# willis-richard/connect4

Hardware: AMD Instinct MI355X
Metric: mcts_node_expansions_per_sec (higher is better)
Workload: dtype f32x3

## Files before the change

### connect4_amd/csrc/c4_engine.hip

```cpp
#include <hip/hip_runtime.h>
#include <hip/hip_fp16.h>
#include <hip/hip_bfloat16.h>

#include <algorithm>
#include <cmath>
#include <cstdarg>
#include <cstdio>
#include <cstdlib>
#include <cstring>
#include <limits>
#include <vector>

#include "../../include/c4_engine.h"
#include "c4_board.h"
#include "c4_net_dev.h"

#ifndef C4_DEADLINE_EVERY
#define C4_DEADLINE_EVERY 1
#endif
#ifndef C4_TERMQ
#define C4_TERMQ 1
#endif
#ifndef C4_FUSED_NET_STAMPS
#define C4_FUSED_NET_STAMPS 0
#endif
#ifndef C4_ASM_PICK
#define C4_ASM_PICK 1
#endif
#ifndef C4_SPECULATE
#define C4_SPECULATE 1
#endif
#ifndef C4_SPLIT_PHASES
#define C4_SPLIT_PHASES 0
#endif
#ifndef C4_DIV_NORMAL
#define C4_DIV_NORMAL 1
#endif
#ifndef C4_SCORE_ALL
#define C4_SCORE_ALL 1
#endif
#ifndef C4_PATH_ALL_LANES
#define C4_PATH_ALL_LANES 1
#endif
#ifndef C4_PEEL_BACKUP
#define C4_PEEL_BACKUP 1
#endif
#ifndef C4_NO_SUSPEND
#define C4_NO_SUSPEND 1
#endif
#ifndef C4_NET_SANITISES
#define C4_NET_SANITISES 1
#endif
#ifndef C4_WAIT_CLOCK_LAZY
#define C4_WAIT_CLOCK_LAZY 1
#endif
#ifndef C4_SPLIT_PAIRS
#define C4_SPLIT_PAIRS 1
#endif
#ifndef C4_SORT_SLOTS
#define C4_SORT_SLOTS 1
#endif
#ifndef C4_FILLERS
#define C4_FILLERS (C4_ORIENTED_Q && C4_SCORE_ALL)
#endif
#ifndef C4_VGPR_BASES
#define C4_VGPR_BASES 1
#endif
#ifndef C4_ORIENTED_Q
#define C4_ORIENTED_Q 1
#endif
#ifndef C4_COOP_LEGAL
#define C4_COOP_LEGAL 1
#endif
#ifndef C4_PICK_BPERM
#define C4_PICK_BPERM 1
#endif
#ifndef C4_EARLY_REQUEST
#define C4_EARLY_REQUEST 1
#endif

namespace {

using namespace c4;

constexpr int GROUP = 8;
constexpr int SLOTS_PER_BLOCK = 8;
constexpr int BLOCK = GROUP * SLOTS_PER_BLOCK;
constexpr int MAX_DEPTH = 44;

constexpr int SLOT_ACTIVE = 0;
constexpr int SLOT_PARKED = 1;
constexpr int SLOT_MOVE_DONE = 2;

__host__ __device__ __forceinline__ uint32_t pack_info(uint32_t base, uint32_t nchild, uint32_t status,
                                                       uint32_t bit, uint32_t pf64)
{
    return (base >> 3) | (nchild << 19) | (status << 22) | (bit << 25) | (pf64 << 31);
}
__host__ __device__ __forceinline__ uint32_t info_base(uint32_t i) { return (i & 0x7ffffu) << 3; }
__host__ __device__ __forceinline__ uint32_t info_nchild(uint32_t i) { return (i >> 19) & 7u; }
__host__ __device__ __forceinline__ uint32_t info_status(uint32_t i) { return (i >> 22) & 7u; }
__host__ __device__ __forceinline__ uint32_t info_bit(uint32_t i) { return (i >> 25) & 63u; }
__host__ __device__ __forceinline__ uint32_t info_move(uint32_t i) { return info_bit(i) / 7u; }
__host__ __device__ __forceinline__ uint32_t info_pf64(uint32_t i) { return i >> 31; }

struct __attribute__((aligned(16))) PathEntry {
    uint32_t node;
    uint32_t n;
    double w;
};

constexpr int BLOCK_BYTES = 256;
struct __attribute__((aligned(32))) Rec {
    double w;
    double q;
    double p;
    uint32_t n;
    uint32_t info;
};
static_assert(sizeof(Rec) == 32, "node record must be 32 bytes");
struct Pool {
    uint8_t *base;
    __device__ __forceinline__ Rec *rec(uint32_t i) const { return reinterpret_cast<Rec *>(base) + i; }
    __device__ __forceinline__ uint32_t &n(uint32_t i) const { return rec(i)->n; }
    __device__ __forceinline__ uint32_t &info(uint32_t i) const { return rec(i)->info; }
    __device__ __forceinline__ double &w(uint32_t i) const { return rec(i)->w; }
    __device__ __forceinline__ double &q(uint32_t i) const { return rec(i)->q; }
    __device__ __forceinline__ double &p(uint32_t i) const { return rec(i)->p; }
};

struct CacheEntry {
    uint64_t key;
    uint64_t check;
    float value;
    float prior[7];
};
static_assert(sizeof(CacheEntry) == 48, "cache entry must be 48 bytes");

struct SlotStats {
    uint64_t sims, expansions, children, terminal_sims, leaf_evals, depth_sum, moves, games_started,
        games_finished, capped, cache_hits, cache_probes, bad_evals, spec_evals;
};
constexpr int N_STATS = sizeof(SlotStats) / sizeof(uint64_t);

struct SlotMem {
    uint64_t root0, root1, leaf0, leaf1;
    long long gid;
    double root_w;
    uint32_t sims, nalloc;
    int32_t pend;
    uint32_t pdepth, pinfo;
    uint32_t ply;
    uint32_t flags;
    __device__ int state() const { return (int)(flags & 0xffu); }
    __device__ bool has_leaf() const { return ((flags >> 8) & 0xffu) != 0; }
    __device__ int need_root() const { return (int)(flags >> 16); }
    __device__ static uint32_t pack(int state, int has_leaf, int need_root) { return (uint32_t)state | ((uint32_t)has_leaf << 8) | ((uint32_t)need_root << 16); }
};
static_assert(sizeof(SlotMem) == 80, "32 of these must fit the fused kernel's LDS budget");

struct Cold {
    uint32_t *cont_cur, *cont_n;
    double *cont_w;
    int32_t *res_move;
    double *res_value;
    double *res_policy;
    const double *noise_tape;
    const double *u_tape;
    int tape_games;
    uint64_t *stg_c0, *stg_c1;
    int32_t *stg_move;
    double *stg_value;
    double *stg_policy;
    c4_game_record *ring;
    unsigned long long *ring_head, *ring_tail, *dropped;
    unsigned long long *next_game;
    unsigned long long *stamps;
};

struct Dev {
    uint8_t *pool;
    uint64_t *root_c0, *root_c1, *leaf_c0, *leaf_c1;
    int32_t *has_leaf;
    int32_t *pending;
    uint32_t *pending_depth;
    uint32_t *pending_info;
    uint32_t *sims_done;
    uint32_t *n_alloc;
    int32_t *state;
    int32_t *need_root;
    uint32_t *ply;
    long long *game_id;
    PathEntry *path;
    uint64_t *stats;
    const double2 *tabAB;
    CacheEntry *cache;
    const Cold *cold;
    int G;
    int slot_lo, slot_hi;
    uint32_t cap;
    int S;
    int nsm;
    int use_noise;
    int rng_tape;
    int stop_after_move;
    int max_inner;
    int level_budget;
    int time_budget;
    int planes_dtype;
    int rec_cap;
    int cache_bits;
    int has_stamps;
    long long games_target;
    double alpha, frac;
    uint64_t seed;
};

__device__ __forceinline__ double gshfl(double v, int src) { return __shfl(v, src, GROUP); }
__device__ __forceinline__ float gshfl(float v, int src) { return __shfl(v, src, GROUP); }
__device__ __forceinline__ int gshfl(int v, int src) { return __shfl(v, src, GROUP); }
__device__ __forceinline__ uint32_t gshfl(uint32_t v, int src) { return (uint32_t)__shfl((int)v, src, GROUP); }

__device__ __forceinline__ void lds_fence() { asm volatile("s_waitcnt lgkmcnt(0)" ::: "memory"); }
typedef __attribute__((address_space(3))) volatile uint32_t lds_vu32_t;
typedef __attribute__((address_space(3))) volatile float lds_vf32_t;
typedef __attribute__((address_space(3))) volatile uint64_t lds_vu64_t;
__device__ __forceinline__ uint32_t lds_ld(const uint32_t *p) { return *(lds_vu32_t *)p; }
__device__ __forceinline__ void lds_st(uint32_t *p, uint32_t v) { *(lds_vu32_t *)p = v; }
__device__ __forceinline__ float lds_ldf(const float *p) { return *(lds_vf32_t *)p; }
__device__ __forceinline__ void lds_st64(uint64_t *p, uint64_t v) { *(lds_vu64_t *)p = v; }

__device__ __forceinline__ void group_fence()
{
    __builtin_amdgcn_fence(__ATOMIC_RELEASE, "workgroup");
    __builtin_amdgcn_fence(__ATOMIC_ACQUIRE, "workgroup");
}

__device__ __forceinline__ void philox_round(uint32_t c[4], const uint32_t k[2])
{
    const uint64_t p0 = (uint64_t)0xD2511F53u * c[0];
    const uint64_t p1 = (uint64_t)0xCD9E8D57u * c[2];
    const uint32_t n0 = (uint32_t)(p1 >> 32) ^ c[1] ^ k[0];
    const uint32_t n1 = (uint32_t)p1;
    const uint32_t n2 = (uint32_t)(p0 >> 32) ^ c[3] ^ k[1];
    const uint32_t n3 = (uint32_t)p0;
    c[0] = n0; c[1] = n1; c[2] = n2; c[3] = n3;
}
__device__ inline void philox4x32(uint32_t c[4], uint64_t seed)
{
    uint32_t k[2] = {(uint32_t)seed, (uint32_t)(seed >> 32)};
#pragma unroll
    for (int r = 0; r < 10; ++r) {
        philox_round(c, k);
        k[0] += 0x9E3779B9u;
        k[1] += 0xBB67AE85u;
    }
}
__device__ inline void rng_uniform2(uint64_t seed, long long gid, uint32_t ply, uint32_t stream, uint32_t idx,
                                    double &u0, double &u1)
{
    uint32_t c[4] = {(uint32_t)gid, (uint32_t)((uint64_t)gid >> 32), ply * 64u + stream, idx};
    philox4x32(c, seed);
    u0 = (double)((((uint64_t)c[0] << 32) | c[1]) >> 11) * (1.0 / 9007199254740992.0);
    u1 = (double)((((uint64_t)c[2] << 32) | c[3]) >> 11) * (1.0 / 9007199254740992.0);
}
__device__ inline double rng_gamma(uint64_t seed, long long gid, uint32_t ply, uint32_t stream, double alpha)
{
    double u0, u1;
    rng_uniform2(seed, gid, ply, stream, 0, u0, u1);
    double boost = 1.0;
    if (alpha < 1.0) {
        boost = pow(u0 > 0.0 ? u0 : 1e-300, 1.0 / alpha);
        alpha += 1.0;
    }
    const double dd = alpha - 1.0 / 3.0, cc = 1.0 / sqrt(9.0 * dd);
    for (uint32_t it = 1; it <= 24; ++it) {
        double a, b, uu, unused;
        rng_uniform2(seed, gid, ply, stream, 2 * it, a, b);
        rng_uniform2(seed, gid, ply, stream, 2 * it + 1, uu, unused);
        const double x = sqrt(-2.0 * log(a > 0.0 ? a : 1e-300)) * cos(6.283185307179586 * b);
        double v = 1.0 + cc * x;
        if (v <= 0.0) continue;
        v = v * v * v;
        if (uu < 1.0 - 0.0331 * x * x * x * x) return boost * dd * v;
        if (log(uu > 0.0 ? uu : 1e-300) < 0.5 * x * x + dd * (1.0 - v + log(v))) return boost * dd * v;
    }
    return boost * dd;
}

__device__ __forceinline__ double child_value_for(uint32_t status, uint32_t n, double q, int side)
{
    const bool term = status >= ST_XWIN;
#if C4_TERMQ
    const double v = q;
#else
    const double v = term ? 0.5 * (double)(status - ST_XWIN) : q;
#endif
    const double sv = side == 0 ? v : 1.0 - v;
    return (term || n > 0) ? sv : 0.0;
}

__device__ __forceinline__ double orient_q(double v, int parent_side)
{
#if C4_ORIENTED_Q
    return (parent_side & 1) ? 1.0 - v : v;
#else
    (void)parent_side;
    return v;
#endif
}

__device__ __forceinline__ double div_normal(double a, double b)
{
#if C4_DIV_NORMAL
    double r = __builtin_amdgcn_rcp(b);
    double e = __builtin_fma(-b, r, 1.0);
    r = __builtin_fma(r, e, r);
    e = __builtin_fma(-b, r, 1.0);
    r = __builtin_fma(r, e, r);
    const double q = a * r;
    const double rem = __builtin_fma(-b, q, a);
    return __builtin_fma(rem, r, q);
#else
    return a / b;
#endif
}

__device__ __forceinline__ double ucb_score(double A, double B, uint32_t nc, double p, double V, uint32_t pf64)
{
    const double pbc = A * div_normal(B, (double)(nc + 1));
    const double prior_score64 = pbc * p;
    const double s64 = prior_score64 + V;
    const float prior_score32 = (float)pbc * (float)p;
    const float s32 = prior_score32 + (float)V;
    return pf64 ? s64 : (double)s32;
}

__device__ __forceinline__ int legal_mask_group(uint64_t occ)
{
#if C4_COOP_LEGAL
    const int lane = (int)(threadIdx.x & (GROUP - 1));
    const bool legal = lane < WIDTH && col_count(occ, lane < WIDTH ? lane : 0) < HEIGHT;
    const unsigned long long b = __builtin_amdgcn_ballot_w64(legal);
    return (int)((b >> (threadIdx.x & 63u & ~(uint32_t)(GROUP - 1))) & 0x7fu);
#else
    return legal_mask(occ);
#endif
}

__device__ __forceinline__ int group_argmax(double s, int k)
{
#pragma unroll
    for (int m = 1; m < GROUP; m <<= 1) {
        const double os = __shfl_xor(s, m, GROUP);
        const int ok = __shfl_xor(k, m, GROUP);
        if (os > s || (os == s && ok > k)) { s = os; k = ok; }
    }
    return k;
}

template <int CTRL>
__device__ __forceinline__ uint32_t dpp_u32(uint32_t v)
{
    return (uint32_t)__builtin_amdgcn_update_dpp(0, (int)v, CTRL, 0xF, 0xF, true);
}
template <int CTRL>
__device__ __forceinline__ double dpp_f64(double v)
{
    const uint64_t b = (uint64_t)__double_as_longlong(v);
    const uint64_t r = ((uint64_t)dpp_u32<CTRL>((uint32_t)(b >> 32)) << 32) | dpp_u32<CTRL>((uint32_t)b);
    return __longlong_as_double((long long)r);
}
struct Pick {
    double s;
    int k;
    uint32_t n, info;
    double w;
};
#define C4_DPP_SELECT(CTRL)                                                                              \
    asm volatile("s_mov_b64 vcc, %[m]\n"                                                                 \
                 "s_nop 0\n"                                                                             \
                 "v_cndmask_b32_dpp %[n], %[n], %[n], vcc " CTRL " row_mask:0xf bank_mask:0xf\n"         \
                 "v_cndmask_b32_dpp %[i], %[i], %[i], vcc " CTRL " row_mask:0xf bank_mask:0xf\n"         \
                 "v_cndmask_b32_dpp %[wl], %[wl], %[wl], vcc " CTRL " row_mask:0xf bank_mask:0xf\n"      \
                 "v_cndmask_b32_dpp %[wh], %[wh], %[wh], vcc " CTRL " row_mask:0xf bank_mask:0xf\n"      \
                 : [n] "+v"(n), [i] "+v"(info), [wl] "+v"(wl), [wh] "+v"(wh)                              \
                 : [m] "s"(m)                                                                             \
                 : "vcc")
#if C4_ASM_PICK
#define C4_PICK_SELECT(CTRL)                                                                             \
    asm volatile("s_mov_b64 vcc, %[m]\n"                                                                 \
                 "s_nop 0\n"                                                                             \
                 "v_cndmask_b32 %[sl], %[ol], %[sl], vcc\n"                                               \
                 "v_cndmask_b32 %[sh], %[oh], %[sh], vcc\n"                                               \
                 "v_cndmask_b32_dpp %[n], %[n], %[n], vcc " CTRL " row_mask:0xf bank_mask:0xf\n"          \
                 "v_cndmask_b32_dpp %[i], %[i], %[i], vcc " CTRL " row_mask:0xf bank_mask:0xf\n"          \
                 "v_cndmask_b32_dpp %[wl], %[wl], %[wl], vcc " CTRL " row_mask:0xf bank_mask:0xf\n"       \
                 "v_cndmask_b32_dpp %[wh], %[wh], %[wh], vcc " CTRL " row_mask:0xf bank_mask:0xf\n"       \
                 : [sl] "+v"(sl), [sh] "+v"(sh), [n] "+v"(n), [i] "+v"(info), [wl] "+v"(wl), [wh] "+v"(wh) \
                 : [m] "s"(m), [ol] "v"(ol), [oh] "v"(oh)                                                   \
                 : "vcc")
template <int CTRL>
__device__ __forceinline__ void pick_step(double &s, uint32_t &n, uint32_t &info, uint32_t &wl, uint32_t &wh)
{
    const uint64_t sb = (uint64_t)__double_as_longlong(s);
    uint32_t sl = (uint32_t)sb, sh = (uint32_t)(sb >> 32);
    const uint32_t ol = dpp_u32<CTRL>(sl), oh = dpp_u32<CTRL>(sh);
    const double os = __longlong_as_double((long long)(((uint64_t)oh << 32) | ol));
    constexpr unsigned long long HIGH = CTRL == 0xB1 ? 0xAAAAAAAAAAAAAAAAull : (CTRL == 0x4E ? 0xCCCCCCCCCCCCCCCCull : 0xF0F0F0F0F0F0F0F0ull);
    const unsigned long long m = __builtin_amdgcn_fcmp(s, os, 2 ) | (__builtin_amdgcn_fcmp(s, os, 3 ) & HIGH);
    if (CTRL == 0xB1) C4_PICK_SELECT("quad_perm:[1,0,3,2]");
    else if (CTRL == 0x4E) C4_PICK_SELECT("quad_perm:[2,3,0,1]");
    else C4_PICK_SELECT("row_half_mirror");
    s = __longlong_as_double((long long)(((uint64_t)sh << 32) | sl));
}
#undef C4_PICK_SELECT
#else
template <int CTRL>
__device__ __forceinline__ void pick_step(double &s, int &k, uint32_t &n, uint32_t &info, uint32_t &wl, uint32_t &wh)
{
    const double os = dpp_f64<CTRL>(s);
    const int ok = (int)dpp_u32<CTRL>((uint32_t)k);
    const bool keep = (s > os) | ((s == os) & (k >= ok));
    s = keep ? s : os;
    k = keep ? k : ok;
    const unsigned long long m = __builtin_amdgcn_ballot_w64(keep);
    if (CTRL == 0xB1) C4_DPP_SELECT("quad_perm:[1,0,3,2]");
    else if (CTRL == 0x4E) C4_DPP_SELECT("quad_perm:[2,3,0,1]");
    else C4_DPP_SELECT("row_half_mirror");
}
#endif
#undef C4_DPP_SELECT
#if C4_PICK_BPERM
__device__ __forceinline__ void group_pick(Pick &a)
{
    double m = a.s, o;
    o = dpp_f64<0xB1>(m);
    asm("v_max_f64 %0, %1, %2" : "=v"(m) : "v"(m), "v"(o));
    o = dpp_f64<0x4E>(m);
    asm("v_max_f64 %0, %1, %2" : "=v"(m) : "v"(m), "v"(o));
    o = dpp_f64<0x141>(m);
    asm("v_max_f64 %0, %1, %2" : "=v"(m) : "v"(m), "v"(o));
    const unsigned long long eq = __builtin_amdgcn_fcmp(a.s, m, 1 );
    const int gb = (int)(threadIdx.x & 63u & ~(uint32_t)(GROUP - 1));
    const uint32_t bits = (uint32_t)(eq >> gb) & 0xffu;
    const int k = 31 - __builtin_clz(bits);
    const int src = (gb + k) << 2;
    const uint64_t wb = (uint64_t)__double_as_longlong(a.w);
    const uint32_t wl = (uint32_t)__builtin_amdgcn_ds_bpermute(src, (int)(uint32_t)wb), wh = (uint32_t)__builtin_amdgcn_ds_bpermute(src, (int)(uint32_t)(wb >> 32));
    a.n = (uint32_t)__builtin_amdgcn_ds_bpermute(src, (int)a.n);
    a.info = (uint32_t)__builtin_amdgcn_ds_bpermute(src, (int)a.info);
    a.w = __longlong_as_double((long long)(((uint64_t)wh << 32) | wl));
    a.k = k;
    a.s = m;
}
#else
__device__ __forceinline__ void group_pick(Pick &a)
{
    const uint64_t wb = (uint64_t)__double_as_longlong(a.w);
    uint32_t wl = (uint32_t)wb, wh = (uint32_t)(wb >> 32);
#if C4_ASM_PICK
    uint32_t nk = a.n | ((uint32_t)(threadIdx.x & (GROUP - 1)) << 29);
    pick_step<0xB1>(a.s, nk, a.info, wl, wh);
    pick_step<0x4E>(a.s, nk, a.info, wl, wh);
    pick_step<0x141>(a.s, nk, a.info, wl, wh);
    a.k = (int)(nk >> 29);
    a.n = nk & 0x1fffffffu;
#else
    pick_step<0xB1>(a.s, a.k, a.n, a.info, wl, wh);
    pick_step<0x4E>(a.s, a.k, a.n, a.info, wl, wh);
    pick_step<0x141>(a.s, a.k, a.n, a.info, wl, wh);
#endif
    a.w = __longlong_as_double((long long)(((uint64_t)wh << 32) | wl));
}
#endif

__device__ __forceinline__ double dirichlet_from_gamma(double nz, bool legal)
{
    if (!legal) nz = 0.0;
    double s = 0.0;
#pragma unroll
    for (int i = 0; i < 7; ++i) s = s + gshfl(nz, i);
    return nz / s;
}

__device__ __forceinline__ int sample_child_sq(double V, bool act, uint32_t nc, double u, int lane)
{
    const double w2 = act ? V * V : 0.0;
    double s2 = 0.0;
#pragma unroll
    for (int i = 0; i < 7; ++i) s2 = s2 + gshfl(w2, i);
    if (!(s2 > 0.0)) return -1;
    const double pk = w2 / s2;
    double acc = 0.0, cdf = 0.0;
#pragma unroll
    for (int i = 0; i < 7; ++i) {
        acc = acc + gshfl(pk, i);
        if (i == lane) cdf = acc;
    }
    const double last = gshfl(cdf, (int)nc - 1);
    cdf = cdf / last;
    const unsigned long long bal = __ballot(act && cdf <= u);
    const int cnt = __popcll((bal >> (((threadIdx.x & 63) / GROUP) * GROUP)) & 0xffull);
    return cnt < (int)nc ? cnt : (int)nc - 1;
}

template <class DevT>
__device__ __forceinline__ void publish_game(DevT &d, int g, long long gid, int len, int32_t result, int lane)
{
    group_fence();
    int ok = 0;
    unsigned long long t = 0;
    if (lane == 0) {
        const unsigned long long tail = *(volatile unsigned long long *)d.cold->ring_tail;
        unsigned long long old = *(volatile unsigned long long *)d.cold->ring_head;
        for (;;) {
            if (old - tail >= (unsigned long long)d.rec_cap) { atomicAdd(d.cold->dropped, 1ULL); break; }
            const unsigned long long seen = atomicCAS(d.cold->ring_head, old, old + 1);
            if (seen == old) { ok = 1; t = old; break; }
            old = seen;
        }
    }
    ok = gshfl(ok, 0);
    if (!ok) return;
    t = ((unsigned long long)gshfl((uint32_t)(t >> 32), 0) << 32) | gshfl((uint32_t)t, 0);
    c4_game_record *row = d.cold->ring + (size_t)(t % (unsigned long long)d.rec_cap);
    const size_t s0 = (size_t)g * 42;
    for (int i = lane; i < len; i += GROUP) {
        row->color0[i] = d.cold->stg_c0[s0 + i];
        row->color1[i] = d.cold->stg_c1[s0 + i];
        row->move[i] = d.cold->stg_move[s0 + i];
        row->value[i] = d.cold->stg_value[s0 + i];
    }
// ... 892 lines not shown
        const int nleaf = sn;
        for (int r0 = 0; r0 < nleaf; r0 += P) {
            if (r0) __syncthreads();
            net_forward_block(nd, NetLds{act, wbuf, mlp}, sleaf[0] + r0, sleaf[1] + r0, min(P, nleaf - r0), 0, s_val, s_pri,
                              smap + r0);
        }
        __syncthreads();
        if (d.has_stamps) t_net += __builtin_amdgcn_s_memtime() - tc;
    }
    if (threadIdx.x < TS && slot0 + threadIdx.x < d.G) {
        const int p = threadIdx.x, g = slot0 + p;
        const SlotMem m = smem[p];
        d.root_c0[g] = m.root0; d.root_c1[g] = m.root1; d.leaf_c0[g] = m.leaf0; d.leaf_c1[g] = m.leaf1;
        d.game_id[g] = m.gid; d.sims_done[g] = m.sims; d.n_alloc[g] = m.nalloc; d.pending[g] = m.pend;
        d.pending_depth[g] = m.pdepth; d.pending_info[g] = m.pinfo; d.need_root[g] = m.need_root();
        d.ply[g] = m.ply; d.state[g] = m.state(); d.has_leaf[g] = m.has_leaf() ? 1 : 0;
    }
    if (threadIdx.x < N_STATS) d.stats[(size_t)slot0 * N_STATS + threadIdx.x] += s_stats[threadIdx.x];
    for (int i = threadIdx.x; i < TS * 8; i += NTHREADS) {
        const int p = i >> 3, k = i & 7;
        if (slot0 + p < d.G) {
            if (k == 7) values[slot0 + p] = s_val[p];
            else priors[(size_t)(slot0 + p) * 7 + k] = s_pri[p * 7 + k];
        }
    }
    if (d.has_stamps && blockIdx.x < 128 && (threadIdx.x & 63) == 0) {
        unsigned long long *o = d.cold->stamps + blockIdx.x * 16;
        o[wv] = t_own;
        if (wv == 0) { o[8] = t_tree; o[9] = t_net; o[10] = (unsigned long long)n_steps; }
    }
}

typedef __attribute__((address_space(4))) const Dev const_dev;
template <int TS, int MODE>
__global__ __launch_bounds__(c4net::NTHREADS) void c4_selfplay_wave_kernel(const Dev *d_dev, c4net::NetDev nd, float *__restrict__ values,
                                                                           float *__restrict__ priors, int n_steps)
{
    using namespace c4net;
    const_dev &d = *(const_dev *)d_dev;
    constexpr int SPW = TS / NWAVES;
    static_assert(TS % NWAVES == 0 && SPW >= 1 && SPW <= 8, "slots per workgroup");
    constexpr int WBUF = WaveBuf<MODE>::HALVES;
    __shared__ __attribute__((aligned(16))) _Float16 act[NWAVES][WBUF];
    __shared__ __attribute__((aligned(16))) float4 mlp[MLP_F4];
    __shared__ SlotMem smem[TS];
    __shared__ float s_val[TS];
    __shared__ float s_pri[TS * 7];
    __shared__ uint32_t s_stats[N_STATS];
    __shared__ __attribute__((aligned(16))) float s_bias[BIAS_LDS_FLOATS];
    __shared__ __attribute__((aligned(16))) uint16_t s_tab16[64 * TAB16];
    constexpr bool OWN_PATH = MODE == NETMODE_F32_F16;
    __shared__ __attribute__((aligned(16))) PathEntry s_path_own[OWN_PATH ? TS : 1][MAX_DEPTH];
    __shared__ __attribute__((aligned(16))) Rec s_l1_own[OWN_PATH ? TS : 1][GROUP];
    static_assert(OWN_PATH || (sizeof(PathEntry) * MAX_DEPTH + sizeof(Rec) * GROUP) * SPW <= sizeof(_Float16) * WBUF, "a wave's path stacks must fit its activation planes");
    const int slot0 = blockIdx.x * TS;
    const int wv = threadIdx.x >> 6;
    if (threadIdx.x < TS) {
        const int p = threadIdx.x, g = slot0 + p;
        SlotMem m = {};
        m.flags = SlotMem::pack(SLOT_PARKED, 0, 0);
        if (g < d.G) {
            m.root0 = d.root_c0[g]; m.root1 = d.root_c1[g]; m.leaf0 = d.leaf_c0[g]; m.leaf1 = d.leaf_c1[g];
            m.gid = d.game_id[g]; m.sims = d.sims_done[g]; m.nalloc = d.n_alloc[g]; m.pend = d.pending[g];
            m.pdepth = d.pending_depth[g]; m.pinfo = d.pending_info[g];
            m.ply = d.ply[g]; m.flags = SlotMem::pack(d.state[g], d.has_leaf[g], d.need_root[g]);
            m.root_w = *(const double *)(d.pool + (size_t)g * d.cap * (BLOCK_BYTES / 8));
        }
        smem[p] = m;
    }
    if (threadIdx.x < N_STATS) s_stats[threadIdx.x] = 0;
    for (int i = threadIdx.x; i < TS * 8; i += NTHREADS) {
        const int p = i >> 3, k = i & 7;
        const bool ok = slot0 + p < d.G;
        if (k == 7) s_val[p] = ok ? values[slot0 + p] : 0.0f;
        else s_pri[p * 7 + k] = ok ? priors[(size_t)(slot0 + p) * 7 + k] : 0.0f;
    }
    for (int i = threadIdx.x; i < MLP_F4; i += NTHREADS) mlp[i] = nd.mlp[i];
    stage_bias_lds(nd, s_bias);
    if (threadIdx.x < 64) build_tab16<MODE == NETMODE_F64 ? CS64 : CS16>(s_tab16, threadIdx.x);
    if (OWN_PATH)
        for (int i = threadIdx.x; i < TS * MAX_DEPTH; i += NTHREADS) {
            const int p = i / MAX_DEPTH, k = i - p * MAX_DEPTH;
            if (slot0 + p < d.G) s_path_own[p][k] = d.path[(size_t)(slot0 + p) * MAX_DEPTH + k];
        }
    __syncthreads();
    PathEntry (*s_path)[MAX_DEPTH] = OWN_PATH ? s_path_own : reinterpret_cast<PathEntry (*)[MAX_DEPTH]>(&act[wv][0]);
    Rec (*s_l1)[GROUP] = OWN_PATH ? s_l1_own : reinterpret_cast<Rec (*)[GROUP]>(&act[wv][0] + sizeof(PathEntry) * MAX_DEPTH * SPW / sizeof(_Float16));
    unsigned long long t_tree = 0, t_net = 0, n_pass = 0;
    const unsigned long long t_launch = __builtin_amdgcn_s_memtime();
    const unsigned long long quantum = (unsigned long long)n_steps * (unsigned long long)(d.time_budget > 0 ? d.time_budget : 80000);
    while (__builtin_amdgcn_s_memtime() - t_launch < quantum) {
        const unsigned long long ta = d.has_stamps ? __builtin_amdgcn_s_memtime() : 0;
        int tid = threadIdx.x;
        asm volatile("" : "+v"(tid));
        const int lane = tid & (GROUP - 1);
        const int grp = (tid & 63) / GROUP;
        const int sl = (tid >> 6) + NWAVES * grp;
        if (grp < SPW)
            tree_step<C4_EVAL_EXTERNAL_F32, false, true, true, OWN_PATH>(d, slot0 + sl, lane, OWN_PATH ? sl : grp, s_path, s_l1, s_val, s_pri, nullptr,
                                                                         nullptr, &smem[sl], sl, s_stats, t_launch + quantum);
        lds_fence();
        const unsigned long long tb = d.has_stamps ? __builtin_amdgcn_s_memtime() : 0;
        int pend_slot[SPW];
        int cnt = 0;
#pragma unroll
        for (int q = 0; q < SPW; ++q) {
            const int sq = wv + NWAVES * q;
            const int has = __builtin_amdgcn_readfirstlane(smem[sq].has_leaf() ? 1 : 0);
            if (has) pend_slot[cnt++] = sq;
        }
        if (MODE == NETMODE_F32_F16) {
            for (int i = 0; i < cnt; ++i) {
                const int sa = pend_slot[i];
                net_forward_wave16(nd, &act[wv][0], mlp, s_bias, s_tab16, smem[sa].leaf0, smem[sa].leaf1, s_val, s_pri, sa,
                                   (C4_FUSED_NET_STAMPS && d.has_stamps && blockIdx.x < 16) ? d.cold->stamps + 2048 + (blockIdx.x * NWAVES + wv) * 16 : nullptr);
            }
        } else {
            for (int i = 0; i < cnt; ++i) {
                const int sa = pend_slot[i];
                net_forward_wave1_mode<MODE>(nd, &act[wv][0], mlp, s_bias, s_tab16, smem[sa].leaf0, smem[sa].leaf1, s_val, s_pri, sa, nd.w0);
            }
        }
        lds_fence();
        if (d.has_stamps) { t_tree += tb - ta; t_net += __builtin_amdgcn_s_memtime() - tb; n_pass += cnt; }
    }
    if (d.has_stamps && blockIdx.x < 128 && (threadIdx.x & 63) == 0) {
        d.cold->stamps[blockIdx.x * 16 + wv] = t_tree;
        d.cold->stamps[blockIdx.x * 16 + 8 + wv] = t_net | (n_pass << 48);
    }
    __syncthreads();
    if (OWN_PATH)
        for (int i = threadIdx.x; i < TS * MAX_DEPTH; i += NTHREADS) {
            const int p = i / MAX_DEPTH, k = i - p * MAX_DEPTH;
            if (slot0 + p < d.G && smem[p].has_leaf()) d.path[(size_t)(slot0 + p) * MAX_DEPTH + k] = s_path_own[p][k];
        }
    if (threadIdx.x < TS && slot0 + threadIdx.x < d.G) {
        const int p = threadIdx.x, g = slot0 + p;
        const SlotMem m = smem[p];
        d.root_c0[g] = m.root0; d.root_c1[g] = m.root1; d.leaf_c0[g] = m.leaf0; d.leaf_c1[g] = m.leaf1;
        d.game_id[g] = m.gid; d.sims_done[g] = m.sims; d.n_alloc[g] = m.nalloc; d.pending[g] = m.pend;
        d.pending_depth[g] = m.pdepth; d.pending_info[g] = m.pinfo; d.need_root[g] = m.need_root();
        d.ply[g] = m.ply; d.state[g] = m.state(); d.has_leaf[g] = m.has_leaf() ? 1 : 0;
    }
    if (threadIdx.x < N_STATS) d.stats[(size_t)slot0 * N_STATS + threadIdx.x] += s_stats[threadIdx.x];
    for (int i = threadIdx.x; i < TS * 8; i += NTHREADS) {
        const int p = i >> 3, k = i & 7;
        if (slot0 + p < d.G) {
            if (k == 7) values[slot0 + p] = s_val[p];
            else priors[(size_t)(slot0 + p) * 7 + k] = s_pri[p * 7 + k];
        }
    }
}

__device__ __forceinline__ void sanitise_answer(float *s_val, float *s_pri, int row, int lw, uint32_t *wg_stats)
{
    if (lw < GROUP) {
        const float v = s_val[row], p = lw < 7 ? s_pri[row * 7 + lw] : 0.0f;
        const bool bad_v = !(v >= 0.0f && v <= 1.0f), bad_p = !(p >= 0.0f && p <= 3.0e38f);
        if (__builtin_amdgcn_ballot_w64(bad_v || bad_p) & 0xffull) {
            if (bad_v && lw == 0) s_val[row] = 0.5f;
            if (bad_p && lw < 7) s_pri[row * 7 + lw] = 0.0f;
            if (lw == 0) atomicAdd(&wg_stats[offsetof(SlotStats, bad_evals) / sizeof(uint64_t)], 1u);
        }
    }
}

template <int TS, int MODE, int TW = 4>
__global__ __launch_bounds__(c4net::NTHREADS) void c4_selfplay_split_kernel(const Dev *d_dev, c4net::NetDev nd, float *__restrict__ values,
                                                                            float *__restrict__ priors, int n_steps, int spread)
{
    using namespace c4net;
    const_dev &d = *(const_dev *)d_dev;
    constexpr int NW = NWAVES - TW;
    constexpr int SPW = (TS + TW - 1) / TW;
    static_assert(TW >= 1 && NW >= 1 && SPW >= 1 && SPW <= 8 && TS <= 64, "slots per workgroup");
    constexpr bool PAIRS = MODE == NETMODE_F32_F16 && TS == 32 && C4_SPLIT_PAIRS;
    constexpr int WBUF = WaveBuf<MODE>::HALVES * (PAIRS ? 2 : 1);
    constexpr bool SPECULATE = C4_SPECULATE && MODE == NETMODE_F32_F16;
    __shared__ __attribute__((aligned(16))) _Float16 act[NW][WBUF];
    __shared__ __attribute__((aligned(16))) float4 mlp[MLP_F4];
    __shared__ SlotMem smem[TS];
    __shared__ float s_val[TS + NW];
    __shared__ float s_pri[(TS + NW) * 7];
    __shared__ uint32_t s_stats[N_STATS];
    __shared__ __attribute__((aligned(16))) float s_bias[BIAS_LDS_FLOATS];
    __shared__ __attribute__((aligned(16))) uint16_t s_tab16[64 * TAB16];
    __shared__ __attribute__((aligned(16))) half8 s_w0[W0Lds<MODE>::FRAGS];
    __shared__ __attribute__((aligned(16))) PathEntry s_path[TS][MAX_DEPTH];
    __shared__ __attribute__((aligned(16))) Rec s_l1[TS][GROUP];
    __shared__ uint32_t s_req[C4_SPLIT_PHASES ? 3 * TS + 4 : TS];
    __shared__ uint32_t s_simd[4];
    __shared__ uint8_t s_perm[TW * SPW];
    __shared__ uint32_t s_tree_done;
    static_assert(sizeof(act) + sizeof(mlp) + sizeof(smem) + sizeof(s_val) + sizeof(s_pri) + sizeof(s_stats) + sizeof(s_bias) + sizeof(s_tab16) +
                  sizeof(s_w0) + sizeof(s_path) + sizeof(s_l1) + sizeof(s_req) + sizeof(s_simd) + sizeof(s_perm) + 64 <= 160 * 1024,
                  "the split kernel's LDS must fit a CU's 160 KiB");
    const int wg_first = spread ? (int)blockIdx.x : (int)blockIdx.x * TS, wg_stride = spread ? (int)gridDim.x : 1;
    auto gslot = [&](int p) -> int { return wg_first + p * wg_stride; };
    if (threadIdx.x < TS) {
        const int p = threadIdx.x, g = gslot(p);
        SlotMem m = {};
        m.flags = SlotMem::pack(SLOT_PARKED, 0, 0);
        if (g < d.G) {
            m.root0 = d.root_c0[g]; m.root1 = d.root_c1[g]; m.leaf0 = d.leaf_c0[g]; m.leaf1 = d.leaf_c1[g];
            m.gid = d.game_id[g]; m.sims = d.sims_done[g]; m.nalloc = d.n_alloc[g]; m.pend = d.pending[g];
            m.pdepth = d.pending_depth[g]; m.pinfo = d.pending_info[g];
            m.ply = d.ply[g]; m.flags = SlotMem::pack(d.state[g], d.has_leaf[g], d.need_root[g]);
            m.root_w = *(const double *)(d.pool + (size_t)g * d.cap * (BLOCK_BYTES / 8));
        }
        smem[p] = m;
        s_req[p] = m.has_leaf() ? REQ_ANSWERED : REQ_IDLE;
    }
    if (threadIdx.x < N_STATS) s_stats[threadIdx.x] = 0;
    if (threadIdx.x < 4) s_simd[threadIdx.x] = 0;
#if C4_SPLIT_PHASES
    if (threadIdx.x < 4) s_req[3 * TS + threadIdx.x] = 0;
#endif
    if (threadIdx.x == 0) s_tree_done = 0;
    for (int i = threadIdx.x; i < TS * 8; i += NTHREADS) {
        const int p = i >> 3, k = i & 7;
        const int g = gslot(p);
        const bool ok = g < d.G;
        if (k == 7) s_val[p] = ok ? values[g] : 0.0f;
        else s_pri[p * 7 + k] = ok ? priors[(size_t)g * 7 + k] : 0.0f;
    }
    for (int i = threadIdx.x; i < MLP_F4; i += NTHREADS) mlp[i] = nd.mlp[i];
    stage_bias_lds(nd, s_bias);
    if (W0Lds<MODE>::FRAGS > 1) stage_w0_lds(nd, s_w0);
    if (threadIdx.x < 64) build_tab16<WaveRow<MODE>::CS>(s_tab16, threadIdx.x);
    for (int i = threadIdx.x; i < TS * MAX_DEPTH; i += NTHREADS) {
        const int p = i / MAX_DEPTH, k = i - p * MAX_DEPTH;
        if (gslot(p) < d.G) s_path[p][k] = d.path[(size_t)gslot(p) * MAX_DEPTH + k];
    }
    __syncthreads();
    if (C4_SORT_SLOTS && threadIdx.x < 64) {
        const int p = threadIdx.x;
        if (p < TW * SPW) s_perm[p] = 0xff;
        const bool act = p < TS && smem[p < TS ? p : 0].state() == SLOT_ACTIVE;
        const int n_act = __popcll(__builtin_amdgcn_ballot_w64(act));
        if (act) {
            const uint32_t kp = smem[p].ply;
            int rank = 0;
            for (int q = 0; q < TS; ++q)
                if (smem[q].state() == SLOT_ACTIVE) { const uint32_t kq = smem[q].ply; rank += (kq < kp) || (kq == kp && q < p); }
            const int t = (rank * TW) / n_act;
            const int first = (t * n_act + TW - 1) / TW;
            s_perm[t * SPW + (rank - first)] = (uint8_t)p;
        }
    }
    if (C4_NET_SANITISES && threadIdx.x < TS && smem[threadIdx.x].has_leaf()) {
        const int p = threadIdx.x;
        bool bad = false;
        const float v = s_val[p];
        if (!(v >= 0.0f && v <= 1.0f)) { s_val[p] = 0.5f; bad = true; }
        for (int k = 0; k < 7; ++k) {
            const float q = s_pri[p * 7 + k];
            if (!(q >= 0.0f && q <= 3.0e38f)) { s_pri[p * 7 + k] = 0.0f; bad = true; }
        }
        if (bad) atomicAdd(&s_stats[offsetof(SlotStats, bad_evals) / sizeof(uint64_t)], 1u);
    }
    const int simd = (int)__builtin_amdgcn_s_getreg((1 << 11) | (4 << 6) | 4) & 3;
    int rank = 0;
    if ((threadIdx.x & 63) == 0) rank = (int)atomicAdd(&s_simd[simd], 1u);
    rank = __builtin_amdgcn_readfirstlane(rank);
    __syncthreads();
    const bool even = (TW == 4 || TW == 3) && s_simd[0] == 2 && s_simd[1] == 2 && s_simd[2] == 2 && s_simd[3] == 2;
    const int wv = threadIdx.x >> 6;
    const bool is_tree = even ? (rank == 0 && simd < TW) : wv < TW;
    const int role_idx = even ? (is_tree ? simd : (TW == 4 ? simd : (rank == 0 ? 4 : simd))) : (wv < TW ? wv : wv - TW);
    const unsigned long long t_launch = __builtin_amdgcn_s_memtime();
    const unsigned long long quantum = (unsigned long long)n_steps * (unsigned long long)(d.time_budget > 0 ? d.time_budget : 80000);
    unsigned long long t_busy = 0, n_pass = 0;
    if (is_tree) {
        const int tw = role_idx;
        while (__builtin_amdgcn_s_memtime() - t_launch < quantum) {
            const unsigned long long ta = d.has_stamps ? __builtin_amdgcn_s_memtime() : 0;
            int tid = threadIdx.x;
            asm volatile("" : "+v"(tid));
            const int lane = tid & (GROUP - 1);
            const int grp = (tid & 63) / GROUP;
            const int sl0 = tw + TW * grp;
            const int sl = (C4_SORT_SLOTS && grp < SPW) ? (int)s_perm[tw * SPW + grp] : sl0;
            bool runnable = false;
            if (grp < SPW && sl < TS) {
                const uint32_t fl = smem[sl].flags;
                runnable = (fl & 0xffu) == SLOT_ACTIVE && (((fl >> 8) & 0xffu) == 0 || lds_ld(&s_req[sl]) == REQ_ANSWERED);
            }
            if (__builtin_amdgcn_ballot_w64(runnable) == 0) {
                __builtin_amdgcn_s_sleep(8);
                continue;
            }
            if (grp < SPW && sl < TS)
                tree_step<C4_EVAL_EXTERNAL_F32, false, true, true, true, const_dev, true>(d, wg_first + sl * wg_stride, lane, sl, s_path, s_l1, s_val, s_pri, nullptr,
                                                                                          nullptr, &smem[sl], sl, s_stats, t_launch + quantum,
                                                                                          &s_req[sl], TS);
            lds_fence();
            if (d.has_stamps) t_busy += __builtin_amdgcn_s_memtime() - ta;
        }
        if ((threadIdx.x & 63) == 0) atomicAdd(&s_tree_done, 1u);
    } else {
        const int lw = threadIdx.x & 63;
        const int nw = role_idx;
        unsigned long long *const nstamps = (C4_FUSED_NET_STAMPS && d.has_stamps && blockIdx.x < 16) ? d.cold->stamps + 2048 + (blockIdx.x * NWAVES + nw) * 16 : nullptr;
        {
            bool have_spec = false;
            uint64_t sc0 = 0, sc1 = 0;
            for (;;) {
                const uint32_t done = lds_ld(&s_tree_done);
                const uint32_t r = lw < TS ? lds_ld(&s_req[lw]) : REQ_IDLE;
                unsigned long long m = __builtin_amdgcn_ballot_w64(r == REQ_POSTED);
                const int rot = (nw * TS) / NW;
                constexpr unsigned long long ALL = (TS == 64) ? ~0ull : ((1ull << TS) - 1);
                auto first_from = [&](unsigned long long mm) -> int {
                    const unsigned long long mr = ((mm >> rot) | (mm << (TS - rot))) & ALL;
                    return __builtin_amdgcn_readfirstlane((__builtin_ctzll(mr) + rot) % TS);
                };
                auto claim = [&](int slot) -> int {
                    int ok = 0;
                    if (lw == 0) ok = atomicCAS(&s_req[slot], REQ_POSTED, REQ_TAKEN) == REQ_POSTED;
                    return __builtin_amdgcn_readfirstlane(ok);
                };
                int c = -1, c2 = -1, row;
                uint64_t b0, b1;
                if (m != 0) {
                    c = first_from(m);
                    if (!claim(c)) continue;
                    m &= ~(1ull << c);
                    if (PAIRS && m != 0) {
                        c2 = first_from(m);
                        if (!claim(c2)) c2 = -1;
                    }
                    b0 = smem[c].leaf0;
                    b1 = smem[c].leaf1;
                    row = c;
                } else if (SPECULATE && have_spec) {
                    have_spec = false;
                    b0 = sc0;
                    b1 = sc1;
                    row = TS + nw;
                } else {
                    if (done == (uint32_t)TW) break;
                    __builtin_amdgcn_s_sleep(4);
                    continue;
                }
                const bool is_spec = c < 0;
                const unsigned long long ta = d.has_stamps ? __builtin_amdgcn_s_memtime() : 0;
#if C4_SPLIT_PHASES
                const uint32_t t_claim = (uint32_t)__builtin_amdgcn_s_memtime();
                if (!is_spec && lw == 0) { atomicAdd(&s_req[3 * TS + 0], (t_claim - lds_ld(&s_req[TS + c])) >> 6); atomicAdd(&s_req[3 * TS + 3], 1u); }
#endif
                if (PAIRS && c2 >= 0) {
                    const uint64_t a0[2] = {b0, smem[c2].leaf0}, a1[2] = {b1, smem[c2].leaf1};
                    const int o[2] = {c, c2};
                    net_forward_wave16n<2>(nd, &act[nw][0], mlp, s_bias, s_tab16, a0, a1, s_val, s_pri, o);
                } else {
                    net_forward_wave1_mode<MODE>(nd, &act[nw][0], mlp, s_bias, s_tab16, b0, b1, s_val, s_pri, row, s_w0, nstamps);
                }
                lds_fence();
                if (C4_NET_SANITISES) {
                    sanitise_answer(s_val, s_pri, row, lw, s_stats);
                    if (PAIRS && c2 >= 0) sanitise_answer(s_val, s_pri, c2, lw, s_stats);
                    lds_fence();
                }
                if (is_spec) {
                    if (lw < GROUP) cache_insert(d, b0, b1, lw, s_val[row], lw < 7 ? s_pri[row * 7 + lw] : 0.0f);
                    if (lw == 0) atomicAdd(&s_stats[offsetof(SlotStats, spec_evals) / sizeof(uint64_t)], 1u);
                    continue;
                }
                const float ppr = (SPECULATE && lw < 7) ? s_pri[c * 7 + lw] : -1.0f;
                if (lw == 0) {
#if C4_SPLIT_PHASES
                    const uint32_t t_ans = (uint32_t)__builtin_amdgcn_s_memtime();
                    lds_st(&s_req[2 * TS + c], t_ans);
                    atomicAdd(&s_req[3 * TS + 1], (t_ans - t_claim) >> 6);
#endif
                    lds_st(&s_req[c], REQ_ANSWERED);
                    if (PAIRS && c2 >= 0) lds_st(&s_req[c2], REQ_ANSWERED);
                }
                if (PAIRS && c2 >= 0) n_pass += 1;
                if (d.has_stamps) { t_busy += __builtin_amdgcn_s_memtime() - ta; n_pass += 1; }
                if (SPECULATE && !(PAIRS && c2 >= 0) && d.cache != nullptr) {
                    const uint32_t r2 = lw < TS ? lds_ld(&s_req[lw]) : REQ_IDLE;
                    if (__builtin_amdgcn_ballot_w64(r2 == REQ_POSTED) != 0) continue;
                    uint64_t c0 = b0, c1 = b1;
                    int go_spec = 0;
                    if (lw < GROUP) {
                        const int mask = legal_mask(b0 | b1);
                        const bool legal = lw < 7 && ((mask >> lw) & 1);
                        const int kb = group_argmax(legal ? (double)ppr : -1.0, legal ? lw : -1);
                        const uint32_t cst = make_move(c0, c1, kb);
                        float cv, cp;
                        go_spec = (cst < ST_XWIN && !cache_probe(d, c0, c1, lw, cv, cp)) ? 1 : 0;
                    }
                    go_spec = __builtin_amdgcn_readfirstlane(go_spec);
                    if (!go_spec) continue;
                    sc0 = ((uint64_t)(uint32_t)__builtin_amdgcn_readfirstlane((int)(c0 >> 32)) << 32) | (uint32_t)__builtin_amdgcn_readfirstlane((int)c0);
                    sc1 = ((uint64_t)(uint32_t)__builtin_amdgcn_readfirstlane((int)(c1 >> 32)) << 32) | (uint32_t)__builtin_amdgcn_readfirstlane((int)c1);
                    have_spec = true;
                }
            }
        }
    }
    if (!C4_SPLIT_PHASES && d.has_stamps && blockIdx.x < 128 && (threadIdx.x & 63) == 0) {
        d.cold->stamps[blockIdx.x * 16 + (is_tree ? 0 : 8) + role_idx] = t_busy | (n_pass << 48);
        if (TW == 4) d.cold->stamps[blockIdx.x * 16 + (is_tree ? 4 : 12) + role_idx] = (unsigned long long)simd | ((unsigned long long)even << 8);
    }
    __syncthreads();
#if C4_SPLIT_PHASES
    if (d.has_stamps && blockIdx.x < 128 && threadIdx.x < 4) d.cold->stamps[4096 + blockIdx.x * 4 + threadIdx.x] = s_req[3 * TS + threadIdx.x];
#endif
    for (int i = threadIdx.x; i < TS * MAX_DEPTH; i += NTHREADS) {
        const int p = i / MAX_DEPTH, k = i - p * MAX_DEPTH;
        if (gslot(p) < d.G && smem[p].has_leaf()) d.path[(size_t)gslot(p) * MAX_DEPTH + k] = s_path[p][k];
    }
    if (threadIdx.x < TS && gslot(threadIdx.x) < d.G) {
        const int p = threadIdx.x, g = gslot(p);
        const SlotMem m = smem[p];
        d.root_c0[g] = m.root0; d.root_c1[g] = m.root1; d.leaf_c0[g] = m.leaf0; d.leaf_c1[g] = m.leaf1;
        d.game_id[g] = m.gid; d.sims_done[g] = m.sims; d.n_alloc[g] = m.nalloc; d.pending[g] = m.pend;
        d.pending_depth[g] = m.pdepth; d.pending_info[g] = m.pinfo; d.need_root[g] = m.need_root();
        d.ply[g] = m.ply; d.state[g] = m.state(); d.has_leaf[g] = m.has_leaf() ? 1 : 0;
    }
    if (threadIdx.x < N_STATS && wg_first < d.G) d.stats[(size_t)wg_first * N_STATS + threadIdx.x] += s_stats[threadIdx.x];
    for (int i = threadIdx.x; i < TS * 8; i += NTHREADS) {
        const int p = i >> 3, k = i & 7;
        const int g = gslot(p);
        if (g < d.G) {
            if (k == 7) values[g] = s_val[p];
            else priors[(size_t)g * 7 + k] = s_pri[p * 7 + k];
        }
    }
}

__global__ void c4_reset_kernel(Dev d, const uint64_t *c0, const uint64_t *c1, int n_active)
{
    const int g = blockIdx.x * blockDim.x + threadIdx.x;
    if (g >= d.G) return;
    const bool active = g < n_active;
    d.root_c0[g] = (active && c0) ? c0[g] : 0;
    d.root_c1[g] = (active && c1) ? c1[g] : 0;
    d.leaf_c0[g] = 0;
    d.leaf_c1[g] = 0;
    d.has_leaf[g] = 0;
    d.pending[g] = -1;
    d.pending_depth[g] = 0;
    d.pending_info[g] = 0;
    d.sims_done[g] = 0;
    d.n_alloc[g] = 1;
    d.state[g] = active ? SLOT_ACTIVE : SLOT_PARKED;
    d.need_root[g] = active ? 1 : 0;
    d.ply[g] = 0;
    d.game_id[g] = g;
    d.cold->res_move[g] = -1;
    d.cold->res_value[g] = 0.0;
    for (int i = 0; i < 7; ++i) d.cold->res_policy[(size_t)g * 7 + i] = 0.0;
    uint64_t *sp = d.stats + (size_t)g * N_STATS;
    for (int i = 0; i < N_STATS; ++i) sp[i] = 0;
    if (active) sp[offsetof(SlotStats, games_started) / 8] = 1;
    if (g == 0) *d.cold->next_game = (unsigned long long)n_active;
    if (g == 0) { *d.cold->ring_head = 0; *d.cold->ring_tail = 0; *d.cold->dropped = 0; }
}

__global__ void c4_gather_roots_kernel(Dev d, c4_root_result *out)
{
    const int g = blockIdx.x * blockDim.x + threadIdx.x;
    if (g >= d.G) return;
    c4_root_result r;
    memset(&r, 0, sizeof(r));
    const Pool pool{d.pool + (size_t)g * d.cap * (BLOCK_BYTES / 8)};
    r.state = d.state[g];
    r.move = d.cold->res_move[g];
    r.value = d.cold->res_value[g];
    r.color0 = d.root_c0[g];
    r.color1 = d.root_c1[g];
    const uint32_t rinfo = pool.info(0);
    for (int i = 0; i < 7; ++i) { r.child_status[i] = -2; r.values_policy[i] = d.cold->res_policy[(size_t)g * 7 + i]; }
    const uint32_t blocks = d.n_alloc[g] < d.cap ? d.n_alloc[g] : d.cap;
    const uint32_t rcb = info_base(rinfo);
    if (info_status(rinfo) == ST_EVALUATED && rcb >= GROUP && rcb + GROUP <= blocks * GROUP) {
        r.root_visits = pool.n(0);
        r.root_value_sum = pool.w(0);
        const uint32_t cb = rcb, nc = info_nchild(rinfo);
        for (uint32_t k = 0; k < nc; ++k) {
            const uint32_t ci = pool.info(cb + k);
            const int m = (int)info_move(ci);
            if (m >= 7) continue;
            r.child_visits[m] = pool.n(cb + k);
            r.child_value_sum[m] = pool.w(cb + k);
            r.child_status[m] = info_status(ci) >= ST_XWIN ? (int32_t)(info_status(ci) - ST_XWIN) : -1;
            r.root_prior[m] = pool.p(cb + k);
        }
    }
    const uint64_t *sp = d.stats + (size_t)g * N_STATS;
    r.expansions = (int64_t)sp[offsetof(SlotStats, expansions) / 8];
    r.simulations = (int64_t)sp[offsetof(SlotStats, sims) / 8];
    out[g] = r;
}

__global__ void k_make_move(const uint64_t *c0, const uint64_t *c1, const int32_t *col, int n, uint64_t *o0,
                            uint64_t *o1, int32_t *res)
{
    const int i = blockIdx.x * blockDim.x + threadIdx.x;
    if (i >= n) return;
    uint64_t a = c0[i], b = c1[i];
    const uint32_t st = make_move(a, b, col[i]);
    o0[i] = a;
    o1[i] = b;
    res[i] = st >= ST_XWIN ? (int32_t)(st - ST_XWIN) : C4_RESULT_NONE;
}
__global__ void k_wins(const uint64_t *s, int n, int32_t *out)
{
    const int i = blockIdx.x * blockDim.x + threadIdx.x;
    if (i < n) out[i] = wins(s[i]) ? 1 : 0;
}
__global__ void k_valid_mask(const uint64_t *c0, const uint64_t *c1, int n, int32_t *out)
{
    const int i = blockIdx.x * blockDim.x + threadIdx.x;
    if (i >= n) return;
    out[i] = position_status(c0[i], c1[i]) == ST_FRESH ? legal_mask(c0[i] | c1[i]) : 0;
}
__global__ void k_planes(const uint64_t *c0, const uint64_t *c1, int n, float *out)
{
    const size_t t = (size_t)blockIdx.x * blockDim.x + threadIdx.x;
    if (t >= (size_t)n * 126) return;
    const size_t i = t / 126;
    const int e = (int)(t - i * 126);
    const int o_to_move = (popc64(c0[i] | c1[i]) & 1) ? 0 : 1;
    out[t] = plane_element(c0[i], c1[i], o_to_move, e);
}
__global__ void k_fliplr(const uint64_t *c0, const uint64_t *c1, int n, uint64_t *o0, uint64_t *o1)
{
    const int i = blockIdx.x * blockDim.x + threadIdx.x;
    if (i >= n) return;
    o0[i] = flip_color(c0[i]);
    o1[i] = flip_color(c1[i]);
}
__global__ void k_centre(const uint64_t *c0, const uint64_t *c1, int n, double *out)
{
    const int i = blockIdx.x * blockDim.x + threadIdx.x;
    if (i < n) out[i] = centre_value(c0[i], c1[i]);
}

__global__ void k_count_active(const int32_t *state, int G, int32_t *out)
{
    __shared__ int total;
    if (threadIdx.x == 0) total = 0;
    __syncthreads();
    int c = 0;
    for (int g = threadIdx.x; g < G; g += blockDim.x) c += state[g] == SLOT_ACTIVE ? 1 : 0;
    atomicAdd(&total, c);
    __syncthreads();
    if (threadIdx.x == 0) *out = total;
}

constexpr int EXPORT_OFFS = 4;
__global__ __launch_bounds__(1024) void k_export_scan(const Cold *cold, int rec_cap, int max_games, long long cap_pos, int64_t *scratch)
{
    __shared__ long long part[1024];
    __shared__ long long base;
    __shared__ int n_ok;
    const int tid = threadIdx.x;
    const unsigned long long head = *cold->ring_head, tail = *cold->ring_tail;
    long long avail = (long long)(head - tail);
    if (avail > max_games) avail = max_games;
    if (tid == 0) { base = 0; n_ok = 0; }
    __syncthreads();
    for (long long chunk = 0; chunk < avail; chunk += 1024) {
        const long long i = chunk + tid;
        const long long len = i < avail ? cold->ring[(tail + (unsigned long long)i) % (unsigned long long)rec_cap].length : 0;
        part[tid] = len;
        __syncthreads();
        for (int o = 1; o < 1024; o <<= 1) {
            const long long v = tid >= o ? part[tid - o] : 0;
            __syncthreads();
            part[tid] += v;
            __syncthreads();
        }
        const long long incl = base + part[tid];
        if (i < avail) {
            scratch[EXPORT_OFFS + i] = incl - len;
            if (incl <= cap_pos) atomicMax(&n_ok, (int)(i + 1));
        }
        __syncthreads();
        if (tid == 0) base += part[1023];
        __syncthreads();
    }
    if (tid == 0) {
        const int n = n_ok;
        scratch[0] = n;
        scratch[1] = n ? scratch[EXPORT_OFFS + n - 1] + cold->ring[(tail + (unsigned long long)(n - 1)) % (unsigned long long)rec_cap].length : 0;
        scratch[2] = (int64_t)tail;
    }
}
__global__ __launch_bounds__(64) void k_export_write(const Cold *cold, int rec_cap, const int64_t *scratch, c4_export_buffers b)
{
    const long long n = scratch[0];
    const unsigned long long tail = (unsigned long long)scratch[2];
    const int t = threadIdx.x;
    for (long long i = blockIdx.x; i < n; i += gridDim.x) {
        const c4_game_record *row = cold->ring + (size_t)((tail + (unsigned long long)i) % (unsigned long long)rec_cap);
        const int len = row->length;
        const long long p = scratch[EXPORT_OFFS + i] + t;
        if (t < len) {
            if (b.boards_dev) { b.boards_dev[2 * p] = (int64_t)row->color0[t]; b.boards_dev[2 * p + 1] = (int64_t)row->color1[t]; }
            if (b.moves_dev) b.moves_dev[p] = (uint8_t)row->move[t];
            if (b.values_dev) b.values_dev[p] = (float)row->value[t];
            if (b.targets_dev) b.targets_dev[p] = 0.5f * (float)row->result;
            if (b.policy_dev)
                for (int k = 0; k < 7; ++k) b.policy_dev[p * 7 + k] = (float)row->policy[t][k];
            if (b.game_index_dev) b.game_index_dev[p] = (int32_t)i;
        }
        if (t == 0) {
            if (b.lengths_dev) b.lengths_dev[i] = len;
            if (b.results_dev) b.results_dev[i] = (int8_t)row->result;
            if (b.ids_dev) b.ids_dev[i] = row->game_id;
        }
    }
}
__global__ void k_export_commit(const Cold *cold, const int64_t *scratch, int64_t *counts_out)
{
    *cold->ring_tail = (unsigned long long)(scratch[2] + scratch[0]);
    if (counts_out) { counts_out[0] = scratch[0]; counts_out[1] = scratch[1]; }
}

__global__ void k_training_tensors(const int64_t *boards, const float *targets, const float *policy, long long n, int flip,
                                   float *ob, float *ov, float *op)
{
    const long long t = (long long)blockIdx.x * blockDim.x + threadIdx.x;
    const long long total = n * (flip ? 2 : 1);
    if (t >= total * 126) return;
    const long long j = t / 126;
    const int e = (int)(t - j * 126);
    const bool mirrored = j >= n;
    const long long src = mirrored ? j - n : j;
    uint64_t c0 = (uint64_t)boards[2 * src], c1 = (uint64_t)boards[2 * src + 1];
    if (mirrored) { c0 = flip_color(c0); c1 = flip_color(c1); }
    const int o_to_move = (popc64(c0 | c1) & 1) ? 0 : 1;
    ob[t] = plane_element(c0, c1, o_to_move, e);
    if (e < 7) op[j * 7 + e] = policy[src * 7 + (mirrored ? 6 - e : e)];
    if (e == 7) ov[j] = targets[src];
}

__global__ __launch_bounds__(64) void k_cache_lookup(Dev d, const uint64_t *c0, const uint64_t *c1, int n, float *value, float *prior,
                                                     int32_t *found)
{
    const int lane = threadIdx.x & (GROUP - 1);
    const int idx = (blockIdx.x * 64 + threadIdx.x) / GROUP;
    const int i = idx < n ? idx : n - 1;
    float v, pl;
    const bool hit = cache_probe(d, c0[i], c1[i], lane, v, pl);
    if (idx < n) {
        if (lane < 7) prior[(size_t)i * 7 + lane] = hit ? pl : 0.0f;
        if (lane == 0) { value[i] = hit ? v : 0.0f; found[i] = hit ? 1 : 0; }
    }
}

__global__ __launch_bounds__(64) void k_debug_noise(uint64_t seed, double alpha, const long long *gid, const int32_t *ply,
                                                    const int32_t *legal_mask, int n, double *raw, double *dirichlet)
{
    const int lane = threadIdx.x & (GROUP - 1);
    const int idx = (blockIdx.x * 64 + threadIdx.x) / GROUP;
    const int i = idx < n ? idx : n - 1;
// ... 1126 lines not shown
```

### connect4_amd/csrc/c4_net_dev.h

```cpp
#pragma once
#include <type_traits>
#include <hip/hip_runtime.h>

#include <cstdint>
#include <vector>

namespace c4net {

typedef _Float16 half8 __attribute__((ext_vector_type(8)));
typedef _Float16 half4 __attribute__((ext_vector_type(4)));
typedef float floatx16 __attribute__((ext_vector_type(16)));

constexpr int F = 32;
constexpr int P = 16;
constexpr int PIX = 42;
constexpr int ROWS = P * PIX;
constexpr int TILES = ROWS / 32;
constexpr int CS = 40;
constexpr int KSTEPS = 18;
constexpr int NWAVES = 8;
constexpr int NTHREADS = NWAVES * 64;
constexpr int WCHUNKS = KSTEPS * 64;
constexpr int HEADV = 3 * PIX;
constexpr int HSTR = 128;
// ... 415 lines not shown
    if (n_layers > 0) {
#pragma unroll
        for (int i = 0; i < 18; ++i) w[i] = nd.conv_w16[i * 64 + lane];
    }
    half8 sw[4];
#pragma unroll
    for (int i = 0; i < 4; ++i) sw[i] = nd.stem_w16[i * 64 + lane];
    const half8 hw = nd.head_w16[lane];
    const float hb0 = nd.head_b[0], hb1 = nd.head_b[1], hb2 = nd.head_b[2];
    uint32_t tb[TAB16 / 2];
    {
        const uint4 *t4 = reinterpret_cast<const uint4 *>(tab + lane * TAB16);
#pragma unroll
        for (int i = 0; i < TAB16 / 8; ++i) { const uint4 v = t4[i]; tb[4 * i] = v.x; tb[4 * i + 1] = v.y; tb[4 * i + 2] = v.z; tb[4 * i + 3] = v.w; }
    }
    auto tof = [&](int idx) -> int { return (int)((tb[idx >> 1] >> (16 * (idx & 1))) & 0xffffu); };
#pragma unroll
    for (int i = 0; i < NP; ++i) {
        _Float16 *inp = P1(i);
        if (lane <= PIX) {
            half4 v = {};
            if (lane < PIX) {
                const int y = lane / 7, x = lane - y * 7;
                const int bit = x * 7 + (5 - y);
                v[0] = (_Float16)((__popcll(b0[i] | b1[i]) & 1) ? 0.0f : 1.0f);
                v[1] = (_Float16)(float)((b0[i] >> bit) & 1);
                v[2] = (_Float16)(float)((b1[i] >> bit) & 1);
            }
            *reinterpret_cast<half4 *>(inp + lane * 4) = v;
        }
        if (lane < CS16) { P0(i)[PIX * CS16 + lane] = (_Float16)0.0f; P1(i)[PIX * CS16 + lane] = (_Float16)0.0f; }
    }
    bool real[RT16];
    int rbase[RT16];
#pragma unroll
    for (int rt = 0; rt < RT16; ++rt) {
        real[rt] = 16 * rt + n < PIX;
        rbase[rt] = (real[rt] ? 16 * rt + n : PIX) * CS16;
    }
    auto bias4 = [&](const float *b, int ct) -> floatx4 {
        const float4 v = *reinterpret_cast<const float4 *>(b + 16 * ct + 4 * g);
        return floatx4{v.x, v.y, v.z, v.w};
    };
    {
        floatx4 acc[NP][RT16][2];
#pragma unroll
        for (int ct = 0; ct < 2; ++ct) {
            const floatx4 bv = bias4(bias_lds, ct);
#pragma unroll
            for (int i = 0; i < NP; ++i)
#pragma unroll
                for (int rt = 0; rt < RT16; ++rt) acc[i][rt][ct] = bv;
        }
#pragma unroll
        for (int s = 0; s < 2; ++s)
#pragma unroll
            for (int i = 0; i < NP; ++i)
#pragma unroll
                for (int rt = 0; rt < RT16; ++rt) {
                    const half4 va = *reinterpret_cast<const half4 *>(P1(i) + tof(27 + rt * 4 + s * 2));
                    const half4 vb = *reinterpret_cast<const half4 *>(P1(i) + tof(27 + rt * 4 + s * 2 + 1));
                    half8 bf;
#pragma unroll
                    for (int j = 0; j < 4; ++j) { bf[j] = va[j]; bf[4 + j] = vb[j]; }
#pragma unroll
                    for (int ct = 0; ct < 2; ++ct) acc[i][rt][ct] = __builtin_amdgcn_mfma_f32_16x16x32_f16(sw[s * 2 + ct], bf, acc[i][rt][ct], 0, 0, 0);
                }
#pragma unroll
        for (int i = 0; i < NP; ++i)
#pragma unroll
            for (int rt = 0; rt < RT16; ++rt)
#pragma unroll
                for (int ct = 0; ct < 2; ++ct) store16(acc[i][rt][ct], P0(i), rbase[rt] + 16 * ct + 4 * g, real[rt]);
    }
    stamp(1);
    auto layer = [&](auto second_tag, const int L) {
        constexpr bool second = decltype(second_tag)::value;
        constexpr int so = second ? PLANE16 : 0, dofs = second ? 0 : PLANE16;
        floatx4 acc[NP][RT16][2];
#pragma unroll
        for (int ct = 0; ct < 2; ++ct) {
            const floatx4 bv = bias4(bias_lds + F * (1 + L), ct);
#pragma unroll
            for (int i = 0; i < NP; ++i)
#pragma unroll
                for (int rt = 0; rt < RT16; ++rt) acc[i][rt][ct] = bv;
        }
        const int Ln = L + 1 < n_layers ? L + 1 : 0;
        const half8 *wnext = nd.conv_w16 + (size_t)Ln * 18 * 64 + lane;
        half8 bf[BDEPTH][NP][RT16];
#pragma unroll
        for (int t = 0; t < BDEPTH - 1; ++t)
#pragma unroll
            for (int i = 0; i < NP; ++i)
#pragma unroll
                for (int rt = 0; rt < RT16; ++rt) bf[t][i][rt] = *reinterpret_cast<const half8 *>(P0(i) + so + tof(rt * 9 + t));
#pragma unroll
        for (int t = 0; t < 9; ++t) {
            if (t + BDEPTH - 1 < 9) {
#pragma unroll
                for (int i = 0; i < NP; ++i)
#pragma unroll
                    for (int rt = 0; rt < RT16; ++rt)
                        bf[(t + BDEPTH - 1) % BDEPTH][i][rt] = *reinterpret_cast<const half8 *>(P0(i) + so + tof(rt * 9 + t + BDEPTH - 1));
            }
#pragma unroll
            for (int ct = 0; ct < 2; ++ct) {
#pragma unroll
                for (int i = 0; i < NP; ++i)
#pragma unroll
                    for (int rt = 0; rt < RT16; ++rt)
                        acc[i][rt][ct] = __builtin_amdgcn_mfma_f32_16x16x32_f16(w[2 * t + ct], bf[t % BDEPTH][i][rt], acc[i][rt][ct], 0, 0, 0);
                w[2 * t + ct] = wnext[(2 * t + ct) * 64];
            }
        }
        if (L == C4_NET_STAMP_LAYER) stamp(12);
        if (second) {
#pragma unroll
            for (int i = 0; i < NP; ++i)
#pragma unroll
                for (int rt = 0; rt < RT16; ++rt) {
                    const half8 x = *reinterpret_cast<const half8 *>(P0(i) + dofs + rbase[rt] + 8 * g);
#pragma unroll
                    for (int ct = 0; ct < 2; ++ct) {
                        half8 idf;
#pragma unroll
                        for (int j = 0; j < 8; ++j) idf[j] = (_Float16)((8 * g + j) == 16 * ct + n ? 1.0f : 0.0f);
                        acc[i][rt][ct] = __builtin_amdgcn_mfma_f32_16x16x32_f16(idf, x, acc[i][rt][ct], 0, 0, 0);
                    }
                }
        }
        if (L == C4_NET_STAMP_LAYER) stamp(13);
#pragma unroll
        for (int i = 0; i < NP; ++i)
#pragma unroll
            for (int rt = 0; rt < RT16; ++rt)
#pragma unroll
                for (int ct = 0; ct < 2; ++ct) store16(acc[i][rt][ct], P0(i) + dofs, rbase[rt] + 16 * ct + 4 * g, real[rt]);
        if (L == C4_NET_STAMP_LAYER) stamp(14);
        if (L < 6) stamp(2 + L);
    };
    for (int blk = 0; blk < nd.n_res; ++blk) {
        layer(std::false_type{}, 2 * blk);
        layer(std::true_type{}, 2 * blk + 1);
    }
    stamp(8);
#pragma unroll
    for (int i = 0; i < NP; ++i) {
    float *hs = reinterpret_cast<float *>(P1(i));
    {
        floatx4 a[RT16];
#pragma unroll
        for (int rt = 0; rt < RT16; ++rt) {
            const half8 x = *reinterpret_cast<const half8 *>(P0(i) + rbase[rt] + 8 * g);
            a[rt] = __builtin_amdgcn_mfma_f32_16x16x32_f16(hw, x, floatx4{0.0f, 0.0f, 0.0f, 0.0f}, 0, 0, 0);
        }
#pragma unroll
        for (int rt = 0; rt < RT16; ++rt) {
            const int r = 16 * rt + n;
            if (g == 0 && r < PIX) {
                hs[0 * PIX + r] = lrelu(a[rt][0] + hb0);
                hs[1 * PIX + r] = lrelu(a[rt][1] + hb1);
                hs[2 * PIX + r] = lrelu(a[rt][2] + hb2);
            }
        }
        if (lane < 2) hs[HEADV + lane] = 0.0f;
    }
    if (i == NP - 1) stamp(9);
    {
        const float *vt_b = reinterpret_cast<const float *>(mlp + VT_F4 + PT_F / 4);
        const float *pt = reinterpret_cast<const float *>(mlp + VT_F4);
        const float4 *hA4 = reinterpret_cast<const float4 *>(hs);
        float v0 = 0.0f;
#pragma unroll
        for (int q = 0; q < 11; ++q) {
            const float4 wv = mlp[q * 64 + lane];
            const float4 xa = hA4[q];
            v0 += wv.x * xa.x + wv.y * xa.y + wv.z * xa.z + wv.w * xa.w;
        }
        const int seg = lane >> 3;
        const float *hpA = hs + PIX + seg * 11;
        float l0 = 0.0f;
#pragma unroll
        for (int c = 0; c < 11; ++c) {
            const float wv = pt[c * 64 + lane];
            const int cc = seg * 11 + c < 2 * PIX ? c : 2 * PIX - 1 - seg * 11;
            l0 += wv * hpA[cc];
        }
        l0 += dppf<0x128>(l0);
#pragma unroll
        for (int m = 16; m <= 32; m <<= 1) l0 += __shfl_xor(l0, m, 64);
        const float fb = vt_b[lane], vw = vt_b[64 + lane], pb = vt_b[128 + lane];
        const bool is_pol = lane < 7;
        const float a = v0 + fb;
        const float lg = l0 + pb;
        const float rs = sum16(lane < PIX ? vw * lrelu(a) : 0.0f);
        const float vsum = readlane_f(rs, 0) + readlane_f(rs, 16) + readlane_f(rs, 32);
        const float value = (tanhf(vsum + nd.vout_b) + nd.w1) * nd.w2;
        const float mx = max8(is_pol ? lg : -INFINITY);
        const float e = is_pol ? expf(lg - mx) : 0.0f;
        const float sum = sum8(e);
        if (lane == 0) values[out[i]] = value;
        if (is_pol) priors[(size_t)out[i] * 7 + lane] = e / sum;
    }
    }
    stamp(10);
#undef P0
#undef P1
}

__device__ __forceinline__ void net_forward_wave16(const NetDev &nd, _Float16 *buf, const float4 *mlp, const float *bias_lds,
                                                   const uint16_t *tab, uint64_t b0, uint64_t b1, float *__restrict__ values,
                                                   float *__restrict__ priors, int out, unsigned long long *stamps = nullptr)
{
    const uint64_t a0[1] = {b0}, a1[1] = {b1};
    const int o[1] = {out};
    net_forward_wave16n<1>(nd, buf, mlp, bias_lds, tab, a0, a1, values, priors, o, stamps);
}

constexpr int WTAPS = 3;

__device__ __forceinline__ void store16p(const floatx4 &hi, const floatx4 &lo, _Float16 *dh, _Float16 *dl, int off, bool real)
{
    half4 oh, ol;
#pragma unroll
    for (int i = 0; i < 4; ++i) {
        const float y = lrelu(hi[i] + lo[i] * LO_INV);
        const _Float16 yh = (_Float16)y;
        oh[i] = yh;
        ol[i] = (_Float16)((y - (float)yh) * LO_SCALE);
    }
    if (real) {
        *reinterpret_cast<half4 *>(dh + off) = oh;
        *reinterpret_cast<half4 *>(dl + off) = ol;
    }
}

#ifndef C4_F32X3_SGB
#define C4_F32X3_SGB 1
#endif
#ifndef C4_F32X3_PKEPI
#define C4_F32X3_PKEPI 1
#endif
#ifndef C4_F32X3_MIXEPI
#define C4_F32X3_MIXEPI 1
#endif
typedef unsigned int u32x4 __attribute__((ext_vector_type(4)));
typedef float float2v __attribute__((ext_vector_type(2)));
typedef _Float16 half2v __attribute__((ext_vector_type(2)));

constexpr int W0_STEM = 0, W0_HEAD = 8, W0_TOWER = 10, W0_FRAGS = 18;
__device__ __forceinline__ half8 wq_load(const __amdgpu_buffer_rsrc_t &r, int voff, int soff)
{
    const u32x4 v = __builtin_amdgcn_raw_buffer_load_b128(r, voff, soff, 0);
    return __builtin_bit_cast(half8, v);
}
__device__ __forceinline__ __amdgpu_buffer_rsrc_t wq_rsrc(const NetDev &nd)
{
    return __builtin_amdgcn_make_buffer_rsrc((void *)nd.conv_w16p, 0, (int)nd.conv_w16p_bytes, 0x00020000);
}
__device__ __forceinline__ void stage_w0_lds(const NetDev &nd, half8 *w0)
{
    for (int i = threadIdx.x; i < W0_FRAGS * 64; i += blockDim.x) w0[i] = nd.w0[i];
}

__device__ __forceinline__ void store16q(const floatx4 &hi, const floatx4 &lo, _Float16 *dh, _Float16 *dl, int off, bool real)
{
#if C4_F32X3_PKEPI
    half4 oh, ol;
#pragma unroll
    for (int i = 0; i < 2; ++i) {
        const float2v h = {hi[2 * i], hi[2 * i + 1]}, l = {lo[2 * i], lo[2 * i + 1]};
        const float2v inv = {LO_INV, LO_INV}, leak = {LEAK, LEAK}, sc = {LO_SCALE, LO_SCALE};
        float2v y = __builtin_elementwise_fma(l, inv, h);
        const float2v ly = y * leak;
        asm("v_max_f32 %0, %1, %2" : "=v"(y.x) : "v"(y.x), "v"(ly.x));
        asm("v_max_f32 %0, %1, %2" : "=v"(y.y) : "v"(y.y), "v"(ly.y));
        const half2v yh = __builtin_convertvector(y, half2v);
#if C4_F32X3_MIXEPI
        const float2v ysc = y * sc;
        const uint32_t yhb = __builtin_bit_cast(uint32_t, yh);
        const float nsc = -LO_SCALE;
        uint32_t ylb;
        asm("v_fma_mixlo_f16 %0, %1, %2, %3 op_sel:[0,0,0] op_sel_hi:[1,0,0]" : "=v"(ylb) : "v"(yhb), "s"(nsc), "v"(ysc.x));
        asm("v_fma_mixhi_f16 %0, %1, %2, %3 op_sel:[1,0,0] op_sel_hi:[1,0,0]" : "+v"(ylb) : "v"(yhb), "s"(nsc), "v"(ysc.y));
        const half2v yl = __builtin_bit_cast(half2v, ylb);
#else
        const float2v back = __builtin_convertvector(yh, float2v);
        const float2v rl = (y - back) * sc;
        const half2v yl = __builtin_convertvector(rl, half2v);
#endif
        oh[2 * i] = yh.x; oh[2 * i + 1] = yh.y;
        ol[2 * i] = yl.x; ol[2 * i + 1] = yl.y;
    }
    if (real) {
        *reinterpret_cast<half4 *>(dh + off) = oh;
        *reinterpret_cast<half4 *>(dl + off) = ol;
    }
#else
    store16p(hi, lo, dh, dl, off, real);
#endif
}

__device__ __forceinline__ void net_forward_wave16q(const NetDev &nd, _Float16 *buf, const float4 *mlp, const float *bias_lds,
                                                    const uint16_t *tab, uint64_t b0, uint64_t b1, float *__restrict__ values,
                                                    float *__restrict__ priors, int out, const half8 *w0, unsigned long long *stamps = nullptr)
{
    int lane_ = threadIdx.x & 63;
    asm volatile("" : "+v"(lane_));
    const int lane = lane_;
    const int n = lane & 15, g = lane >> 4;
    auto stamp = [&](int i) { if (stamps && lane == 0) stamps[i] = __builtin_amdgcn_s_memtime(); };
    stamp(0);
    _Float16 *const p0h = buf, *const p0l = buf + PLANE16, *const p1h = buf + 2 * PLANE16, *const p1l = buf + 3 * PLANE16;
    const __amdgpu_buffer_rsrc_t wr = wq_rsrc(nd);
    const int voff = lane * 16;
    int soff = 2 * 4096;
    half8 wh[WTAPS][2], wl[WTAPS][2];
#pragma unroll
    for (int t = 0; t < 2; ++t)
#pragma unroll
        for (int ct = 0; ct < 2; ++ct) {
            wh[t][ct] = w0[(W0_TOWER + t * 4 + 2 * ct) * 64 + lane];
            wl[t][ct] = w0[(W0_TOWER + t * 4 + 2 * ct + 1) * 64 + lane];
        }
#pragma unroll
    for (int ct = 0; ct < 2; ++ct) { wh[2][ct] = wh[0][ct]; wl[2][ct] = wl[0][ct]; }
    half8 swh[4], swl[4];
#pragma unroll
    for (int i = 0; i < 4; ++i) { swh[i] = w0[(W0_STEM + i) * 64 + lane]; swl[i] = w0[(W0_STEM + 4 + i) * 64 + lane]; }
    const float hb0 = nd.head_b[0], hb1 = nd.head_b[1], hb2 = nd.head_b[2];
    uint32_t tb[TAB16 / 2];
    {
        const uint4 *t4 = reinterpret_cast<const uint4 *>(tab + lane * TAB16);
#pragma unroll
        for (int i = 0; i < TAB16 / 8; ++i) { const uint4 v = t4[i]; tb[4 * i] = v.x; tb[4 * i + 1] = v.y; tb[4 * i + 2] = v.z; tb[4 * i + 3] = v.w; }
    }
    auto tof = [&](int idx) -> int { return (int)((tb[idx >> 1] >> (16 * (idx & 1))) & 0xffffu); };
    _Float16 *inp = p1h;
    if (lane <= PIX) {
        half4 v = {};
        if (lane < PIX) {
            const int y = lane / 7, x = lane - y * 7;
            const int bit = x * 7 + (5 - y);
            v[0] = (_Float16)((__popcll(b0 | b1) & 1) ? 0.0f : 1.0f);
            v[1] = (_Float16)(float)((b0 >> bit) & 1);
            v[2] = (_Float16)(float)((b1 >> bit) & 1);
        }
        *reinterpret_cast<half4 *>(inp + lane * 4) = v;
    }
    if (lane < CS16) {
        p0h[PIX * CS16 + lane] = (_Float16)0.0f; p0l[PIX * CS16 + lane] = (_Float16)0.0f;
        p1h[PIX * CS16 + lane] = (_Float16)0.0f; p1l[PIX * CS16 + lane] = (_Float16)0.0f;
    }
    bool real[RT16];
    int rbase[RT16];
#pragma unroll
    for (int rt = 0; rt < RT16; ++rt) {
        real[rt] = 16 * rt + n < PIX;
        rbase[rt] = (real[rt] ? 16 * rt + n : PIX) * CS16;
    }
    auto bias4 = [&](const float *b, int ct) -> floatx4 {
        const float4 v = *reinterpret_cast<const float4 *>(b + 16 * ct + 4 * g);
        return floatx4{v.x, v.y, v.z, v.w};
    };
    const floatx4 zero4 = {0.0f, 0.0f, 0.0f, 0.0f};
    {
        floatx4 ah[RT16][2], al[RT16][2];
#pragma unroll
        for (int ct = 0; ct < 2; ++ct) {
            const floatx4 bv = bias4(bias_lds, ct);
#pragma unroll
            for (int rt = 0; rt < RT16; ++rt) { ah[rt][ct] = bv; al[rt][ct] = zero4; }
        }
#pragma unroll
        for (int s = 0; s < 2; ++s)
#pragma unroll
            for (int rt = 0; rt < RT16; ++rt) {
                const half4 va = *reinterpret_cast<const half4 *>(inp + tof(27 + rt * 4 + s * 2));
                const half4 vb = *reinterpret_cast<const half4 *>(inp + tof(27 + rt * 4 + s * 2 + 1));
                half8 bf;
#pragma unroll
                for (int j = 0; j < 4; ++j) { bf[j] = va[j]; bf[4 + j] = vb[j]; }
#pragma unroll
                for (int ct = 0; ct < 2; ++ct) {
                    ah[rt][ct] = __builtin_amdgcn_mfma_f32_16x16x32_f16(swh[s * 2 + ct], bf, ah[rt][ct], 0, 0, 0);
                    al[rt][ct] = __builtin_amdgcn_mfma_f32_16x16x32_f16(swl[s * 2 + ct], bf, al[rt][ct], 0, 0, 0);
                }
            }
#pragma unroll
        for (int rt = 0; rt < RT16; ++rt)
#pragma unroll
            for (int ct = 0; ct < 2; ++ct) store16q(ah[rt][ct], al[rt][ct], p0h, p0l, rbase[rt] + 16 * ct + 4 * g, real[rt]);
    }
    stamp(1);
    auto layer = [&](auto second_tag, const int L) {
        constexpr bool second = decltype(second_tag)::value;
        const _Float16 *sh = second ? p1h : p0h, *sl = second ? p1l : p0l;
        _Float16 *dh = second ? p0h : p1h, *dl = second ? p0l : p1l;
        floatx4 ah[RT16][2], al[RT16][2];
#pragma unroll
        for (int ct = 0; ct < 2; ++ct) {
            const floatx4 bv = bias4(bias_lds + F * (1 + L), ct);
#pragma unroll
            for (int rt = 0; rt < RT16; ++rt) { ah[rt][ct] = bv; al[rt][ct] = zero4; }
        }
        half8 bh[RT16], bl[RT16], nh[RT16], nl[RT16];
#pragma unroll
        for (int rt = 0; rt < RT16; ++rt) {
            bh[rt] = *reinterpret_cast<const half8 *>(sh + tof(rt * 9));
            bl[rt] = *reinterpret_cast<const half8 *>(sl + tof(rt * 9));
        }
#if C4_F32X3_SGB
        __builtin_amdgcn_sched_barrier(0);
#endif
#pragma unroll
        for (int t = 0; t < 9; ++t) {
            {
#pragma unroll
                for (int ct = 0; ct < 2; ++ct) {
                    wh[(t + 2) % WTAPS][ct] = wq_load(wr, voff + (2 * ct) * 1024, soff);
                    wl[(t + 2) % WTAPS][ct] = wq_load(wr, voff + (2 * ct + 1) * 1024, soff);
                }
                soff += 4096;
            }
            if (t + 1 < 9) {
#pragma unroll
                for (int rt = 0; rt < RT16; ++rt) {
                    nh[rt] = *reinterpret_cast<const half8 *>(sh + tof(rt * 9 + t + 1));
                    nl[rt] = *reinterpret_cast<const half8 *>(sl + tof(rt * 9 + t + 1));
                }
            }
#pragma unroll
            for (int ct = 0; ct < 2; ++ct) {
                const half8 cwh = wh[t % WTAPS][ct], cwl = wl[t % WTAPS][ct];
#pragma unroll
                for (int rt = 0; rt < RT16; ++rt) {
                    ah[rt][ct] = __builtin_amdgcn_mfma_f32_16x16x32_f16(cwh, bh[rt], ah[rt][ct], 0, 0, 0);
                    al[rt][ct] = __builtin_amdgcn_mfma_f32_16x16x32_f16(cwl, bh[rt], al[rt][ct], 0, 0, 0);
                    al[rt][ct] = __builtin_amdgcn_mfma_f32_16x16x32_f16(cwh, bl[rt], al[rt][ct], 0, 0, 0);
                }
            }
#pragma unroll
            for (int rt = 0; rt < RT16; ++rt) { bh[rt] = nh[rt]; bl[rt] = nl[rt]; }
#if C4_F32X3_SGB
#pragma unroll
            for (int i = 0; i < 4; ++i) { __builtin_amdgcn_sched_group_barrier(0x008, 1, 0); __builtin_amdgcn_sched_group_barrier(0x020, 1, 0); }
            if (t + 1 < 9) {
#pragma unroll
                for (int i = 0; i < 6; ++i) { __builtin_amdgcn_sched_group_barrier(0x008, 2, 0); __builtin_amdgcn_sched_group_barrier(0x100, 1, 0); }
                __builtin_amdgcn_sched_group_barrier(0x008, 2, 0);
            } else {
                __builtin_amdgcn_sched_group_barrier(0x008, 14, 0);
            }
#endif
        }
#if C4_F32X3_SGB
        __builtin_amdgcn_sched_barrier(0);
#endif
        if (L == C4_NET_STAMP_LAYER) stamp(12);
        if (second) {
#pragma unroll
            for (int rt = 0; rt < RT16; ++rt) {
                const half8 xh = *reinterpret_cast<const half8 *>(dh + rbase[rt] + 8 * g);
                const half8 xl = *reinterpret_cast<const half8 *>(dl + rbase[rt] + 8 * g);
#pragma unroll
                for (int ct = 0; ct < 2; ++ct) {
                    half8 idf;
#pragma unroll
                    for (int j = 0; j < 8; ++j) idf[j] = (_Float16)((8 * g + j) == 16 * ct + n ? 1.0f : 0.0f);
                    ah[rt][ct] = __builtin_amdgcn_mfma_f32_16x16x32_f16(idf, xh, ah[rt][ct], 0, 0, 0);
                    al[rt][ct] = __builtin_amdgcn_mfma_f32_16x16x32_f16(idf, xl, al[rt][ct], 0, 0, 0);
                }
            }
        }
        if (L == C4_NET_STAMP_LAYER) stamp(13);
#pragma unroll
        for (int rt = 0; rt < RT16; ++rt)
#pragma unroll
            for (int ct = 0; ct < 2; ++ct) store16q(ah[rt][ct], al[rt][ct], dh, dl, rbase[rt] + 16 * ct + 4 * g, real[rt]);
        if (L == C4_NET_STAMP_LAYER) stamp(14);
        if (L < 6) stamp(2 + L);
    };
    for (int blk = 0; blk < nd.n_res; ++blk) {
        layer(std::false_type{}, 2 * blk);
        layer(std::true_type{}, 2 * blk + 1);
    }
    stamp(8);
    float *hs = reinterpret_cast<float *>(p1h);
    {
        const half8 hwh = w0[W0_HEAD * 64 + lane], hwl = w0[(W0_HEAD + 1) * 64 + lane];
        floatx4 a[RT16], b[RT16];
#pragma unroll
        for (int rt = 0; rt < RT16; ++rt) {
            const half8 xh = *reinterpret_cast<const half8 *>(p0h + rbase[rt] + 8 * g);
            const half8 xl = *reinterpret_cast<const half8 *>(p0l + rbase[rt] + 8 * g);
            a[rt] = __builtin_amdgcn_mfma_f32_16x16x32_f16(hwh, xh, zero4, 0, 0, 0);
            b[rt] = __builtin_amdgcn_mfma_f32_16x16x32_f16(hwl, xh, zero4, 0, 0, 0);
            b[rt] = __builtin_amdgcn_mfma_f32_16x16x32_f16(hwh, xl, b[rt], 0, 0, 0);
        }
#pragma unroll
        for (int rt = 0; rt < RT16; ++rt) {
            const int r = 16 * rt + n;
            if (g == 0 && r < PIX) {
                hs[0 * PIX + r] = lrelu(a[rt][0] + b[rt][0] * LO_INV + hb0);
                hs[1 * PIX + r] = lrelu(a[rt][1] + b[rt][1] * LO_INV + hb1);
                hs[2 * PIX + r] = lrelu(a[rt][2] + b[rt][2] * LO_INV + hb2);
            }
        }
        if (lane < 2) hs[HEADV + lane] = 0.0f;
    }
    stamp(9);
    {
        const float *vt_b = reinterpret_cast<const float *>(mlp + VT_F4 + PT_F / 4);
        const float *pt = reinterpret_cast<const float *>(mlp + VT_F4);
        const float4 *hA4 = reinterpret_cast<const float4 *>(hs);
        float v0 = 0.0f;
#pragma unroll
        for (int q = 0; q < 11; ++q) {
            const float4 wv = mlp[q * 64 + lane];
            const float4 xa = hA4[q];
            v0 += wv.x * xa.x + wv.y * xa.y + wv.z * xa.z + wv.w * xa.w;
        }
        const int seg = lane >> 3;
        const float *hpA = hs + PIX + seg * 11;
        float l0 = 0.0f;
#pragma unroll
        for (int cc0 = 0; cc0 < 11; ++cc0) {
            const float wv = pt[cc0 * 64 + lane];
            const int cc = seg * 11 + cc0 < 2 * PIX ? cc0 : 2 * PIX - 1 - seg * 11;
            l0 += wv * hpA[cc];
        }
        l0 += dppf<0x128>(l0);
#pragma unroll
        for (int m = 16; m <= 32; m <<= 1) l0 += __shfl_xor(l0, m, 64);
        const float fb = vt_b[lane], vw = vt_b[64 + lane], pb = vt_b[128 + lane];
        const bool is_pol = lane < 7;
        const float a = v0 + fb;
        const float lg = l0 + pb;
        const float rs = sum16(lane < PIX ? vw * lrelu(a) : 0.0f);
        const float vsum = readlane_f(rs, 0) + readlane_f(rs, 16) + readlane_f(rs, 32);
        const float value = (tanhf(vsum + nd.vout_b) + nd.w1) * nd.w2;
        const float mx = max8(is_pol ? lg : -INFINITY);
        const float e = is_pol ? expf(lg - mx) : 0.0f;
        const float sum = sum8(e);
        if (lane == 0) values[out] = value;
        if (is_pol) priors[(size_t)out * 7 + lane] = e / sum;
    }
    stamp(10);
}

constexpr int CS64 = 72;
constexpr int PLANE64 = PROWS * CS64;
constexpr int WUNITS = 3;

__device__ __forceinline__ void net_forward_wave16w(const NetDev &nd, _Float16 *buf, const float4 *mlp, const float *bias_lds,
                                                    const uint16_t *tab, uint64_t b0, uint64_t b1, float *__restrict__ values,
                                                    float *__restrict__ priors, int out, unsigned long long *stamps = nullptr)
{
    constexpr int FW = 64, CT = 4, KS = 2;
    int lane_ = threadIdx.x & 63;
    asm volatile("" : "+v"(lane_));
    const int lane = lane_;
    const int n = lane & 15, g = lane >> 4;
    auto stamp = [&](int i) { if (stamps && lane == 0) stamps[i] = __builtin_amdgcn_s_memtime(); };
    stamp(0);
    const int n_layers = 2 * nd.n_res;
    _Float16 *const p0 = buf, *const p1 = buf + PLANE64;
    half8 w[WUNITS][CT];
    const half8 *wp = nd.conv_w16 + lane;
    const int total_units = n_layers * 18;
#pragma unroll
    for (int u = 0; u < WUNITS; ++u) {
        const int U = u < total_units ? u : 0;
#pragma unroll
        for (int ct = 0; ct < CT; ++ct) w[u][ct] = wp[(U * CT + ct) * 64];
    }
    half8 sw[2][CT];
#pragma unroll
    for (int s = 0; s < 2; ++s)
#pragma unroll
        for (int ct = 0; ct < CT; ++ct) sw[s][ct] = nd.stem_w16[(s * CT + ct) * 64 + lane];
    const half8 hw0 = nd.head_w16[lane], hw1 = nd.head_w16[64 + lane];
    const float hb0 = nd.head_b[0], hb1 = nd.head_b[1], hb2 = nd.head_b[2];
    uint32_t tb[TAB16 / 2];
    {
        const uint4 *t4 = reinterpret_cast<const uint4 *>(tab + lane * TAB16);
#pragma unroll
        for (int i = 0; i < TAB16 / 8; ++i) { const uint4 v = t4[i]; tb[4 * i] = v.x; tb[4 * i + 1] = v.y; tb[4 * i + 2] = v.z; tb[4 * i + 3] = v.w; }
    }
    auto tof = [&](int idx) -> int { return (int)((tb[idx >> 1] >> (16 * (idx & 1))) & 0xffffu); };
    _Float16 *inp = p1;
    if (lane <= PIX) {
        half4 v = {};
        if (lane < PIX) {
            const int y = lane / 7, x = lane - y * 7;
            const int bit = x * 7 + (5 - y);
            v[0] = (_Float16)((__popcll(b0 | b1) & 1) ? 0.0f : 1.0f);
            v[1] = (_Float16)(float)((b0 >> bit) & 1);
            v[2] = (_Float16)(float)((b1 >> bit) & 1);
        }
        *reinterpret_cast<half4 *>(inp + lane * 4) = v;
    }
    for (int i = lane; i < CS64; i += 64) { p0[PIX * CS64 + i] = (_Float16)0.0f; p1[PIX * CS64 + i] = (_Float16)0.0f; }
    bool real[RT16];
    int rbase[RT16];
#pragma unroll
    for (int rt = 0; rt < RT16; ++rt) {
        real[rt] = 16 * rt + n < PIX;
        rbase[rt] = (real[rt] ? 16 * rt + n : PIX) * CS64;
    }
    auto bias4 = [&](const float *b, int ct) -> floatx4 {
        const float4 v = *reinterpret_cast<const float4 *>(b + 16 * ct + 4 * g);
        return floatx4{v.x, v.y, v.z, v.w};
    };
    {
        floatx4 acc[RT16][CT];
#pragma unroll
        for (int ct = 0; ct < CT; ++ct) {
            const floatx4 bv = bias4(bias_lds, ct);
#pragma unroll
            for (int rt = 0; rt < RT16; ++rt) acc[rt][ct] = bv;
        }
#pragma unroll
        for (int s = 0; s < 2; ++s)
#pragma unroll
            for (int rt = 0; rt < RT16; ++rt) {
                const half4 va = *reinterpret_cast<const half4 *>(inp + tof(27 + rt * 4 + s * 2));
                const half4 vb = *reinterpret_cast<const half4 *>(inp + tof(27 + rt * 4 + s * 2 + 1));
                half8 bf;
#pragma unroll
                for (int j = 0; j < 4; ++j) { bf[j] = va[j]; bf[4 + j] = vb[j]; }
#pragma unroll
                for (int ct = 0; ct < CT; ++ct) acc[rt][ct] = __builtin_amdgcn_mfma_f32_16x16x32_f16(sw[s][ct], bf, acc[rt][ct], 0, 0, 0);
            }
#pragma unroll
        for (int rt = 0; rt < RT16; ++rt)
#pragma unroll
            for (int ct = 0; ct < CT; ++ct) store16(acc[rt][ct], p0, rbase[rt] + 16 * ct + 4 * g, real[rt]);
    }
    stamp(1);
    auto layer = [&](auto second_tag, const int L) {
        constexpr bool second = decltype(second_tag)::value;
        const _Float16 *src = second ? p1 : p0;
        _Float16 *dst = second ? p0 : p1;
        floatx4 acc[RT16][CT];
#pragma unroll
        for (int ct = 0; ct < CT; ++ct) {
            const floatx4 bv = bias4(bias_lds + FW * (1 + L), ct);
#pragma unroll
            for (int rt = 0; rt < RT16; ++rt) acc[rt][ct] = bv;
        }
        half8 bc[RT16], bn[RT16];
#pragma unroll
        for (int rt = 0; rt < RT16; ++rt) bc[rt] = *reinterpret_cast<const half8 *>(src + tof(rt * 9));
#pragma unroll
        for (int u = 0; u < 18; ++u) {
            if (u + 1 < 18) {
#pragma unroll
                for (int rt = 0; rt < RT16; ++rt) bn[rt] = *reinterpret_cast<const half8 *>(src + tof(rt * 9 + (u + 1) / 2) + 32 * ((u + 1) % 2));
            }
#pragma unroll
            for (int ct = 0; ct < CT; ++ct) {
                const half8 cw = w[u % WUNITS][ct];
#pragma unroll
                for (int rt = 0; rt < RT16; ++rt) acc[rt][ct] = __builtin_amdgcn_mfma_f32_16x16x32_f16(cw, bc[rt], acc[rt][ct], 0, 0, 0);
            }
            {
                int U = L * 18 + u + WUNITS;
                U = U < total_units ? U : 0;
#pragma unroll
                for (int ct = 0; ct < CT; ++ct) w[u % WUNITS][ct] = wp[(U * CT + ct) * 64];
            }
#pragma unroll
            for (int rt = 0; rt < RT16; ++rt) bc[rt] = bn[rt];
        }
        if (second) {
#pragma unroll
            for (int rt = 0; rt < RT16; ++rt)
#pragma unroll
                for (int ks = 0; ks < KS; ++ks) {
                    const half8 x = *reinterpret_cast<const half8 *>(dst + rbase[rt] + 32 * ks + 8 * g);
#pragma unroll
                    for (int c2 = 0; c2 < 2; ++c2) {
                        half8 idf;
#pragma unroll
                        for (int j = 0; j < 8; ++j) idf[j] = (_Float16)((8 * g + j) == 16 * c2 + n ? 1.0f : 0.0f);
                        acc[rt][2 * ks + c2] = __builtin_amdgcn_mfma_f32_16x16x32_f16(idf, x, acc[rt][2 * ks + c2], 0, 0, 0);
                    }
                }
        }
#pragma unroll
        for (int rt = 0; rt < RT16; ++rt)
#pragma unroll
            for (int ct = 0; ct < CT; ++ct) store16(acc[rt][ct], dst, rbase[rt] + 16 * ct + 4 * g, real[rt]);
        if (L < 6) stamp(2 + L);
    };
    for (int blk = 0; blk < nd.n_res; ++blk) {
        layer(std::false_type{}, 2 * blk);
        layer(std::true_type{}, 2 * blk + 1);
    }
    stamp(8);
    float *hs = reinterpret_cast<float *>(p1);
    {
        floatx4 a[RT16];
#pragma unroll
        for (int rt = 0; rt < RT16; ++rt) {
            const half8 x0 = *reinterpret_cast<const half8 *>(p0 + rbase[rt] + 8 * g);
            const half8 x1 = *reinterpret_cast<const half8 *>(p0 + rbase[rt] + 32 + 8 * g);
            a[rt] = __builtin_amdgcn_mfma_f32_16x16x32_f16(hw0, x0, floatx4{0.0f, 0.0f, 0.0f, 0.0f}, 0, 0, 0);
            a[rt] = __builtin_amdgcn_mfma_f32_16x16x32_f16(hw1, x1, a[rt], 0, 0, 0);
        }
#pragma unroll
        for (int rt = 0; rt < RT16; ++rt) {
            const int r = 16 * rt + n;
            if (g == 0 && r < PIX) {
                hs[0 * PIX + r] = lrelu(a[rt][0] + hb0);
                hs[1 * PIX + r] = lrelu(a[rt][1] + hb1);
                hs[2 * PIX + r] = lrelu(a[rt][2] + hb2);
            }
        }
        if (lane < 2) hs[HEADV + lane] = 0.0f;
    }
    stamp(9);
    {
        const float *vt_b = reinterpret_cast<const float *>(mlp + VT_F4 + PT_F / 4);
        const float *pt = reinterpret_cast<const float *>(mlp + VT_F4);
        const float4 *hA4 = reinterpret_cast<const float4 *>(hs);
        float v0 = 0.0f;
#pragma unroll
        for (int q = 0; q < 11; ++q) {
            const float4 wv = mlp[q * 64 + lane];
            const float4 xa = hA4[q];
            v0 += wv.x * xa.x + wv.y * xa.y + wv.z * xa.z + wv.w * xa.w;
        }
        const int seg = lane >> 3;
        const float *hpA = hs + PIX + seg * 11;
        float l0 = 0.0f;
#pragma unroll
        for (int c = 0; c < 11; ++c) {
            const float wv = pt[c * 64 + lane];
            const int cc = seg * 11 + c < 2 * PIX ? c : 2 * PIX - 1 - seg * 11;
            l0 += wv * hpA[cc];
        }
        l0 += dppf<0x128>(l0);
#pragma unroll
        for (int m = 16; m <= 32; m <<= 1) l0 += __shfl_xor(l0, m, 64);
        const float fb = vt_b[lane], vw = vt_b[64 + lane], pb = vt_b[128 + lane];
        const bool is_pol = lane < 7;
        const float a = v0 + fb;
        const float lg = l0 + pb;
        const float rs = sum16(lane < PIX ? vw * lrelu(a) : 0.0f);
        const float vsum = readlane_f(rs, 0) + readlane_f(rs, 16) + readlane_f(rs, 32);
        const float value = (tanhf(vsum + nd.vout_b) + nd.w1) * nd.w2;
        const float mx = max8(is_pol ? lg : -INFINITY);
        const float e = is_pol ? expf(lg - mx) : 0.0f;
        const float sum = sum8(e);
        if (lane == 0) values[out] = value;
        if (is_pol) priors[(size_t)out * 7 + lane] = e / sum;
    }
    stamp(10);
}

__device__ __forceinline__ void net_forward_wave16x(const NetDev &nd, _Float16 *buf, const float4 *mlp, const float *bias_lds,
                                                    const uint16_t *tab, uint64_t b0, uint64_t b1, float *__restrict__ values,
                                                    float *__restrict__ priors, int out, unsigned long long *stamps = nullptr)
{
    constexpr int FW = 64;
    int lane_ = threadIdx.x & 63;
    asm volatile("" : "+v"(lane_));
    const int lane = lane_;
    const int n = lane & 15, g = lane >> 4;
    auto stamp = [&](int i) { if (stamps && lane == 0) stamps[i] = __builtin_amdgcn_s_memtime(); };
    stamp(0);
    _Float16 *const p0h = buf, *const p0l = buf + PLANE64, *const p1h = buf + 2 * PLANE64, *const p1l = buf + 3 * PLANE64;
    const __amdgpu_buffer_rsrc_t wr = wq_rsrc(nd);
    const int voff = lane * 16;
    half8 wh[WTAPS][2], wl[WTAPS][2];
#pragma unroll
    for (int t = 0; t < 2; ++t)
#pragma unroll
        for (int ct = 0; ct < 2; ++ct) {
            wh[t][ct] = wq_load(wr, voff + (2 * ct) * 1024, t * 4096);
            wl[t][ct] = wq_load(wr, voff + (2 * ct + 1) * 1024, t * 4096);
        }
#pragma unroll
    for (int ct = 0; ct < 2; ++ct) { wh[2][ct] = wh[0][ct]; wl[2][ct] = wl[0][ct]; }
    int soff = 2 * 4096;
    const float hb0 = nd.head_b[0], hb1 = nd.head_b[1], hb2 = nd.head_b[2];
    uint32_t tb[TAB16 / 2];
    {
        const uint4 *t4 = reinterpret_cast<const uint4 *>(tab + lane * TAB16);
#pragma unroll
        for (int i = 0; i < TAB16 / 8; ++i) { const uint4 v = t4[i]; tb[4 * i] = v.x; tb[4 * i + 1] = v.y; tb[4 * i + 2] = v.z; tb[4 * i + 3] = v.w; }
    }
    auto tof = [&](int idx) -> int { return (int)((tb[idx >> 1] >> (16 * (idx & 1))) & 0xffffu); };
    _Float16 *inp = p1h;
    if (lane <= PIX) {
        half4 v = {};
        if (lane < PIX) {
            const int y = lane / 7, x = lane - y * 7;
            const int bit = x * 7 + (5 - y);
            v[0] = (_Float16)((__popcll(b0 | b1) & 1) ? 0.0f : 1.0f);
            v[1] = (_Float16)(float)((b0 >> bit) & 1);
            v[2] = (_Float16)(float)((b1 >> bit) & 1);
        }
        *reinterpret_cast<half4 *>(inp + lane * 4) = v;
    }
    for (int i = lane; i < CS64; i += 64) {
        p0h[PIX * CS64 + i] = (_Float16)0.0f; p0l[PIX * CS64 + i] = (_Float16)0.0f;
        p1h[PIX * CS64 + i] = (_Float16)0.0f; p1l[PIX * CS64 + i] = (_Float16)0.0f;
    }
    bool real[RT16];
    int rbase[RT16];
#pragma unroll
    for (int rt = 0; rt < RT16; ++rt) {
        real[rt] = 16 * rt + n < PIX;
        rbase[rt] = (real[rt] ? 16 * rt + n : PIX) * CS64;
    }
    auto bias4 = [&](const float *b, int ct) -> floatx4 {
        const float4 v = *reinterpret_cast<const float4 *>(b + 16 * ct + 4 * g);
        return floatx4{v.x, v.y, v.z, v.w};
    };
    const floatx4 zero4 = {0.0f, 0.0f, 0.0f, 0.0f};
#pragma unroll 1
    for (int ch = 0; ch < 2; ++ch) {
        half8 swh[2][2], swl[2][2];
#pragma unroll
        for (int s = 0; s < 2; ++s)
#pragma unroll
            for (int ct = 0; ct < 2; ++ct) {
                swh[s][ct] = nd.stem_w16[(s * 4 + 2 * ch + ct) * 64 + lane];
                swl[s][ct] = nd.stem_w16l[(s * 4 + 2 * ch + ct) * 64 + lane];
            }
        floatx4 ah[RT16][2], al[RT16][2];
#pragma unroll
        for (int ct = 0; ct < 2; ++ct) {
            const floatx4 bv = bias4(bias_lds + 32 * ch, ct);
#pragma unroll
            for (int rt = 0; rt < RT16; ++rt) { ah[rt][ct] = bv; al[rt][ct] = zero4; }
        }
#pragma unroll
        for (int s = 0; s < 2; ++s)
#pragma unroll
            for (int rt = 0; rt < RT16; ++rt) {
                const half4 va = *reinterpret_cast<const half4 *>(inp + tof(27 + rt * 4 + s * 2));
                const half4 vb = *reinterpret_cast<const half4 *>(inp + tof(27 + rt * 4 + s * 2 + 1));
                half8 bf;
#pragma unroll
                for (int j = 0; j < 4; ++j) { bf[j] = va[j]; bf[4 + j] = vb[j]; }
#pragma unroll
                for (int ct = 0; ct < 2; ++ct) {
                    ah[rt][ct] = __builtin_amdgcn_mfma_f32_16x16x32_f16(swh[s][ct], bf, ah[rt][ct], 0, 0, 0);
                    al[rt][ct] = __builtin_amdgcn_mfma_f32_16x16x32_f16(swl[s][ct], bf, al[rt][ct], 0, 0, 0);
                }
            }
#pragma unroll
        for (int rt = 0; rt < RT16; ++rt)
#pragma unroll
            for (int ct = 0; ct < 2; ++ct) store16q(ah[rt][ct], al[rt][ct], p0h, p0l, rbase[rt] + 32 * ch + 16 * ct + 4 * g, real[rt]);
    }
    stamp(1);
    auto layer = [&](auto second_tag, const int L) {
        constexpr bool second = decltype(second_tag)::value;
        const _Float16 *sh = second ? p1h : p0h, *sl = second ? p1l : p0l;
        _Float16 *dh = second ? p0h : p1h, *dl = second ? p0l : p1l;
#pragma unroll 1
        for (int ch = 0; ch < 2; ++ch) {
            floatx4 ah[RT16][2], al[RT16][2];
#pragma unroll
            for (int ct = 0; ct < 2; ++ct) {
                const floatx4 bv = bias4(bias_lds + FW * (1 + L) + 32 * ch, ct);
#pragma unroll
                for (int rt = 0; rt < RT16; ++rt) { ah[rt][ct] = bv; al[rt][ct] = zero4; }
            }
            half8 bh[RT16], bl[RT16], nh[RT16], nl[RT16];
#pragma unroll
            for (int rt = 0; rt < RT16; ++rt) {
                bh[rt] = *reinterpret_cast<const half8 *>(sh + tof(rt * 9));
                bl[rt] = *reinterpret_cast<const half8 *>(sl + tof(rt * 9));
            }
#if C4_F32X3_SGB
            __builtin_amdgcn_sched_barrier(0);
#endif
#pragma unroll
            for (int u = 0; u < 18; ++u) {
                {
#pragma unroll
                    for (int ct = 0; ct < 2; ++ct) {
                        wh[(u + 2) % WTAPS][ct] = wq_load(wr, voff + (2 * ct) * 1024, soff);
                        wl[(u + 2) % WTAPS][ct] = wq_load(wr, voff + (2 * ct + 1) * 1024, soff);
                    }
                    soff += 4096;
                }
                if (u + 1 < 18) {
#pragma unroll
                    for (int rt = 0; rt < RT16; ++rt) {
                        nh[rt] = *reinterpret_cast<const half8 *>(sh + tof(rt * 9 + (u + 1) / 2) + 32 * ((u + 1) % 2));
                        nl[rt] = *reinterpret_cast<const half8 *>(sl + tof(rt * 9 + (u + 1) / 2) + 32 * ((u + 1) % 2));
                    }
                }
#pragma unroll
                for (int ct = 0; ct < 2; ++ct) {
                    const half8 cwh = wh[u % WTAPS][ct], cwl = wl[u % WTAPS][ct];
#pragma unroll
                    for (int rt = 0; rt < RT16; ++rt) {
                        ah[rt][ct] = __builtin_amdgcn_mfma_f32_16x16x32_f16(cwh, bh[rt], ah[rt][ct], 0, 0, 0);
                        al[rt][ct] = __builtin_amdgcn_mfma_f32_16x16x32_f16(cwl, bh[rt], al[rt][ct], 0, 0, 0);
                        al[rt][ct] = __builtin_amdgcn_mfma_f32_16x16x32_f16(cwh, bl[rt], al[rt][ct], 0, 0, 0);
                    }
                }
#pragma unroll
                for (int rt = 0; rt < RT16; ++rt) { bh[rt] = nh[rt]; bl[rt] = nl[rt]; }
#if C4_F32X3_SGB
#pragma unroll
                for (int i = 0; i < 4; ++i) { __builtin_amdgcn_sched_group_barrier(0x008, 1, 0); __builtin_amdgcn_sched_group_barrier(0x020, 1, 0); }
                if (u + 1 < 18) {
#pragma unroll
                    for (int i = 0; i < 6; ++i) { __builtin_amdgcn_sched_group_barrier(0x008, 2, 0); __builtin_amdgcn_sched_group_barrier(0x100, 1, 0); }
                    __builtin_amdgcn_sched_group_barrier(0x008, 2, 0);
                } else {
                    __builtin_amdgcn_sched_group_barrier(0x008, 14, 0);
                }
#endif
            }
#if C4_F32X3_SGB
            __builtin_amdgcn_sched_barrier(0);
#endif
            if (second) {
#pragma unroll
                for (int rt = 0; rt < RT16; ++rt) {
                    const half8 xh = *reinterpret_cast<const half8 *>(dh + rbase[rt] + 32 * ch + 8 * g);
                    const half8 xl = *reinterpret_cast<const half8 *>(dl + rbase[rt] + 32 * ch + 8 * g);
#pragma unroll
                    for (int ct = 0; ct < 2; ++ct) {
                        half8 idf;
#pragma unroll
                        for (int j = 0; j < 8; ++j) idf[j] = (_Float16)((8 * g + j) == 16 * ct + n ? 1.0f : 0.0f);
                        ah[rt][ct] = __builtin_amdgcn_mfma_f32_16x16x32_f16(idf, xh, ah[rt][ct], 0, 0, 0);
                        al[rt][ct] = __builtin_amdgcn_mfma_f32_16x16x32_f16(idf, xl, al[rt][ct], 0, 0, 0);
                    }
                }
            }
#pragma unroll
            for (int rt = 0; rt < RT16; ++rt)
#pragma unroll
                for (int ct = 0; ct < 2; ++ct) store16q(ah[rt][ct], al[rt][ct], dh, dl, rbase[rt] + 32 * ch + 16 * ct + 4 * g, real[rt]);
        }
        if (L < 6) stamp(2 + L);
    };
    for (int blk = 0; blk < nd.n_res; ++blk) {
        layer(std::false_type{}, 2 * blk);
        layer(std::true_type{}, 2 * blk + 1);
    }
    stamp(8);
    float *hs = reinterpret_cast<float *>(p1h);
    {
        const half8 hwh0 = nd.head_w16[lane], hwh1 = nd.head_w16[64 + lane];
        const half8 hwl0 = nd.head_w16l[lane], hwl1 = nd.head_w16l[64 + lane];
        floatx4 a[RT16], b[RT16];
#pragma unroll
        for (int rt = 0; rt < RT16; ++rt) {
            const half8 xh0 = *reinterpret_cast<const half8 *>(p0h + rbase[rt] + 8 * g);
            const half8 xl0 = *reinterpret_cast<const half8 *>(p0l + rbase[rt] + 8 * g);
            const half8 xh1 = *reinterpret_cast<const half8 *>(p0h + rbase[rt] + 32 + 8 * g);
            const half8 xl1 = *reinterpret_cast<const half8 *>(p0l + rbase[rt] + 32 + 8 * g);
            a[rt] = __builtin_amdgcn_mfma_f32_16x16x32_f16(hwh0, xh0, zero4, 0, 0, 0);
            a[rt] = __builtin_amdgcn_mfma_f32_16x16x32_f16(hwh1, xh1, a[rt], 0, 0, 0);
            b[rt] = __builtin_amdgcn_mfma_f32_16x16x32_f16(hwl0, xh0, zero4, 0, 0, 0);
            b[rt] = __builtin_amdgcn_mfma_f32_16x16x32_f16(hwh0, xl0, b[rt], 0, 0, 0);
            b[rt] = __builtin_amdgcn_mfma_f32_16x16x32_f16(hwl1, xh1, b[rt], 0, 0, 0);
            b[rt] = __builtin_amdgcn_mfma_f32_16x16x32_f16(hwh1, xl1, b[rt], 0, 0, 0);
        }
#pragma unroll
        for (int rt = 0; rt < RT16; ++rt) {
            const int r = 16 * rt + n;
            if (g == 0 && r < PIX) {
                hs[0 * PIX + r] = lrelu(a[rt][0] + b[rt][0] * LO_INV + hb0);
                hs[1 * PIX + r] = lrelu(a[rt][1] + b[rt][1] * LO_INV + hb1);
                hs[2 * PIX + r] = lrelu(a[rt][2] + b[rt][2] * LO_INV + hb2);
            }
        }
        if (lane < 2) hs[HEADV + lane] = 0.0f;
    }
    stamp(9);
    {
        const float *vt_b = reinterpret_cast<const float *>(mlp + VT_F4 + PT_F / 4);
        const float *pt = reinterpret_cast<const float *>(mlp + VT_F4);
        const float4 *hA4 = reinterpret_cast<const float4 *>(hs);
        float v0 = 0.0f;
#pragma unroll
        for (int q = 0; q < 11; ++q) {
            const float4 wv = mlp[q * 64 + lane];
            const float4 xa = hA4[q];
            v0 += wv.x * xa.x + wv.y * xa.y + wv.z * xa.z + wv.w * xa.w;
        }
        const int seg = lane >> 3;
        const float *hpA = hs + PIX + seg * 11;
        float l0 = 0.0f;
#pragma unroll
        for (int c = 0; c < 11; ++c) {
            const float wv = pt[c * 64 + lane];
            const int cc = seg * 11 + c < 2 * PIX ? c : 2 * PIX - 1 - seg * 11;
            l0 += wv * hpA[cc];
        }
        l0 += dppf<0x128>(l0);
#pragma unroll
        for (int m = 16; m <= 32; m <<= 1) l0 += __shfl_xor(l0, m, 64);
        const float fb = vt_b[lane], vw = vt_b[64 + lane], pb = vt_b[128 + lane];
        const bool is_pol = lane < 7;
        const float a = v0 + fb;
        const float lg = l0 + pb;
        const float rs = sum16(lane < PIX ? vw * lrelu(a) : 0.0f);
        const float vsum = readlane_f(rs, 0) + readlane_f(rs, 16) + readlane_f(rs, 32);
        const float value = (tanhf(vsum + nd.vout_b) + nd.w1) * nd.w2;
        const float mx = max8(is_pol ? lg : -INFINITY);
        const float e = is_pol ? expf(lg - mx) : 0.0f;
        const float sum = sum8(e);
        if (lane == 0) values[out] = value;
        if (is_pol) priors[(size_t)out * 7 + lane] = e / sum;
    }
    stamp(10);
}

constexpr int NETMODE_F32_F16 = 0;
constexpr int NETMODE_F32_PRECISE = 1;
constexpr int NETMODE_F64 = 2;
constexpr int NETMODE_F64_PRECISE = 3;
template <int MODE> struct W0Lds { static constexpr int FRAGS = MODE == NETMODE_F32_PRECISE ? W0_FRAGS * 64 : 1; };
template <int MODE>
__device__ __forceinline__ void net_forward_wave1_mode(const NetDev &nd, _Float16 *buf, const float4 *mlp, const float *bias_lds,
                                                       const uint16_t *tab, uint64_t b0, uint64_t b1, float *__restrict__ values,
                                                       float *__restrict__ priors, int out, const half8 *w0,
                                                       unsigned long long *stamps = nullptr)
{
    if constexpr (MODE == NETMODE_F64) net_forward_wave16w(nd, buf, mlp, bias_lds, tab, b0, b1, values, priors, out, stamps);
    else if constexpr (MODE == NETMODE_F64_PRECISE) net_forward_wave16x(nd, buf, mlp, bias_lds, tab, b0, b1, values, priors, out, stamps);
    else if constexpr (MODE == NETMODE_F32_PRECISE) net_forward_wave16q(nd, buf, mlp, bias_lds, tab, b0, b1, values, priors, out, w0, stamps);
    else net_forward_wave16(nd, buf, mlp, bias_lds, tab, b0, b1, values, priors, out, stamps);
}
template <int MODE> struct WaveBuf {
    static constexpr int HALVES = MODE == NETMODE_F64_PRECISE ? 4 * PLANE64
                                  : (MODE == NETMODE_F64 ? 2 * PLANE64 : (MODE == NETMODE_F32_PRECISE ? 4 * PLANE16 : 2 * PLANE16));
};
template <int MODE> struct WaveRow { static constexpr int CS = (MODE == NETMODE_F64 || MODE == NETMODE_F64_PRECISE) ? CS64 : CS16; };

constexpr int BIAS_LDS_FLOATS = 32 * (1 + 32);
__device__ __forceinline__ void stage_bias_lds(const NetDev &nd, float *bias_lds)
{
    const int n_layers = 2 * nd.n_res, fw = nd.filters;
    for (int i = threadIdx.x; i < fw * (1 + n_layers); i += NTHREADS) bias_lds[i] = i < fw ? nd.stem_b[i] : nd.conv_b[i - fw];
}
}

struct c4_net {
    int device;
    c4net::NetDev d;
    std::vector<void *> allocs;
};
```

Baseline: 281.6 million.

## Hoist per-pass net setup into persistent wave state and fuse sanitise into pass

Net waves in the f32x3 precise mode now build a persistent state once per kernel: buffer resource, row bases, head biases, tap table registers, identity fragments and MLP biases. Each evaluation reuses that state instead of recomputing or reloading it. The MLP weights are loaded early so they overlap the head MFMA. The answer sanitise check is folded into the pass, replacing a separate LDS pass and fence, and the leaf board is read speculatively alongside the claim CAS. The cost is a large number of persistent VGPRs (the tap table and identity fragments), which risks register pressure and spills in the conv loop.

Result: no change. 283.7 million (median of 6 runs) (+0.7%).

```diff
diff --git a/connect4_amd/csrc/c4_engine.hip b/connect4_amd/csrc/c4_engine.hip
--- a/connect4_amd/csrc/c4_engine.hip
+++ b/connect4_amd/csrc/c4_engine.hip
@@ -50,6 +50,12 @@
 #endif
 #ifndef C4_NET_SANITISES
 #define C4_NET_SANITISES 1
+#endif
+#ifndef C4_NETPASS_CLAIMREAD
+#define C4_NETPASS_CLAIMREAD 1
+#endif
+#ifndef C4_NETPASS_SANITISE
+#define C4_NETPASS_SANITISE 1
 #endif
 #ifndef C4_WAIT_CLOCK_LAZY
 #define C4_WAIT_CLOCK_LAZY 1
@@ -229,6 +235,7 @@
 __device__ __forceinline__ void lds_st(uint32_t *p, uint32_t v) { *(lds_vu32_t *)p = v; }
 __device__ __forceinline__ float lds_ldf(const float *p) { return *(lds_vf32_t *)p; }
 __device__ __forceinline__ void lds_st64(uint64_t *p, uint64_t v) { *(lds_vu64_t *)p = v; }
+__device__ __forceinline__ uint64_t lds_ld64(const uint64_t *p) { return *(lds_vu64_t *)p; }
 
 __device__ __forceinline__ void group_fence()
 {
@@ -1727,6 +1734,11 @@
         const int lw = threadIdx.x & 63;
         const int nw = role_idx;
         unsigned long long *const nstamps = (C4_FUSED_NET_STAMPS && d.has_stamps && blockIdx.x < 16) ? d.cold->stamps + 2048 + (blockIdx.x * NWAVES + nw) * 16 : nullptr;
+        constexpr bool CARRY = MODE == NETMODE_F32_PRECISE && C4_NETPASS_STATE > 0;
+        constexpr bool CHECK_IN_PASS = CARRY && C4_NETPASS_SANITISE && C4_NET_SANITISES;
+        constexpr bool CLAIM_READS = MODE == NETMODE_F32_PRECISE && C4_NETPASS_CLAIMREAD;
+        Wave16qState nst;
+        if constexpr (CARRY) nst = wave16q_setup<C4_NETPASS_STATE>(nd, &act[nw][0], mlp, s_tab16, s_w0, lw);
         {
             bool have_spec = false;
             uint64_t sc0 = 0, sc1 = 0;
@@ -1749,14 +1761,22 @@
                 uint64_t b0, b1;
                 if (m != 0) {
                     c = first_from(m);
-                    if (!claim(c)) continue;
+                    uint64_t cl0 = 0, cl1 = 0;
+                    if constexpr (CLAIM_READS) {
+                        int won = 0;
+                        if (lw == 0) won = atomicCAS(&s_req[c], REQ_POSTED, REQ_TAKEN) == REQ_POSTED;
+                        asm volatile("" ::: "memory");
+                        cl0 = lds_ld64(&smem[c].leaf0);
+                        cl1 = lds_ld64(&smem[c].leaf1);
+                        if (!__builtin_amdgcn_readfirstlane(won)) continue;
+                    } else if (!claim(c)) continue;
                     m &= ~(1ull << c);
                     if (PAIRS && m != 0) {
                         c2 = first_from(m);
                         if (!claim(c2)) c2 = -1;
                     }
-                    b0 = smem[c].leaf0;
-                    b1 = smem[c].leaf1;
+                    b0 = CLAIM_READS ? cl0 : smem[c].leaf0;
+                    b1 = CLAIM_READS ? cl1 : smem[c].leaf1;
                     row = c;
                 } else if (SPECULATE && have_spec) {
                     have_spec = false;
@@ -1778,11 +1798,14 @@
                     const uint64_t a0[2] = {b0, smem[c2].leaf0}, a1[2] = {b1, smem[c2].leaf1};
                     const int o[2] = {c, c2};
                     net_forward_wave16n<2>(nd, &act[nw][0], mlp, s_bias, s_tab16, a0, a1, s_val, s_pri, o);
+                } else if constexpr (CARRY) {
+                    wave16q_pass<C4_NETPASS_STATE, CHECK_IN_PASS, C4_NETPASS_MLPEARLY != 0>(nst, nd, &act[nw][0], mlp, s_bias, s_tab16, b0, b1, s_val, s_pri, row, s_w0, nstamps,
+                                                                  &s_stats[offsetof(SlotStats, bad_evals) / sizeof(uint64_t)]);
                 } else {
                     net_forward_wave1_mode<MODE>(nd, &act[nw][0], mlp, s_bias, s_tab16, b0, b1, s_val, s_pri, row, s_w0, nstamps);
                 }
                 lds_fence();
-                if (C4_NET_SANITISES) {
+                if (C4_NET_SANITISES && !CHECK_IN_PASS) {
                     sanitise_answer(s_val, s_pri, row, lw, s_stats);
                     if (PAIRS && c2 >= 0) sanitise_answer(s_val, s_pri, c2, lw, s_stats);
                     lds_fence();
diff --git a/connect4_amd/csrc/c4_net_dev.h b/connect4_amd/csrc/c4_net_dev.h
--- a/connect4_amd/csrc/c4_net_dev.h
+++ b/connect4_amd/csrc/c4_net_dev.h
@@ -741,19 +741,79 @@
 #endif
 }
 
-__device__ __forceinline__ void net_forward_wave16q(const NetDev &nd, _Float16 *buf, const float4 *mlp, const float *bias_lds,
-                                                    const uint16_t *tab, uint64_t b0, uint64_t b1, float *__restrict__ values,
-                                                    float *__restrict__ priors, int out, const half8 *w0, unsigned long long *stamps = nullptr)
-{
-    int lane_ = threadIdx.x & 63;
-    asm volatile("" : "+v"(lane_));
-    const int lane = lane_;
+#ifndef C4_NETPASS_STATE
+#define C4_NETPASS_STATE 3
+#endif
+static_assert(C4_NETPASS_STATE >= 0 && C4_NETPASS_STATE <= 3, "C4_NETPASS_STATE: 0 .. 3");
+#ifndef C4_NETPASS_MLPEARLY
+#define C4_NETPASS_MLPEARLY 1
+#endif
+struct Wave16qState {
+    int lane;
+    int voff, rbase[RT16];
+    bool real[RT16];
+    __amdgpu_buffer_rsrc_t wr;
+    float hb0, hb1, hb2, fb, vw, pb;
+    uint32_t tb[TAB16 / 2];
+    half8 idf[2];
+};
+template <int K>
+__device__ __forceinline__ void wave16q_fill(Wave16qState &st, const NetDev &nd, const float4 *mlp, const uint16_t *tab, const half8 *w0)
+{
+    const int lane = st.lane, n = lane & 15, g = lane >> 4;
+    if constexpr (K == 1) {
+        st.wr = wq_rsrc(nd);
+        st.voff = lane * 16;
+        st.hb0 = nd.head_b[0]; st.hb1 = nd.head_b[1]; st.hb2 = nd.head_b[2];
+#pragma unroll
+        for (int rt = 0; rt < RT16; ++rt) {
+            st.real[rt] = 16 * rt + n < PIX;
+            st.rbase[rt] = (st.real[rt] ? 16 * rt + n : PIX) * CS16;
+        }
+    } else if constexpr (K == 6) {
+        const float *vt_b = reinterpret_cast<const float *>(mlp + VT_F4 + PT_F / 4);
+        st.fb = vt_b[lane]; st.vw = vt_b[64 + lane]; st.pb = vt_b[128 + lane];
+    } else if constexpr (K == 2) {
+        const uint4 *t4 = reinterpret_cast<const uint4 *>(tab + lane * TAB16);
+#pragma unroll
+        for (int i = 0; i < TAB16 / 8; ++i) { const uint4 v = t4[i]; st.tb[4 * i] = v.x; st.tb[4 * i + 1] = v.y; st.tb[4 * i + 2] = v.z; st.tb[4 * i + 3] = v.w; }
+    } else {
+        static_assert(K == 3, "state level");
+#pragma unroll
+        for (int ct = 0; ct < 2; ++ct)
+#pragma unroll
+            for (int j = 0; j < 8; ++j) st.idf[ct][j] = (_Float16)((8 * g + j) == 16 * ct + n ? 1.0f : 0.0f);
+    }
+}
+template <int LEVEL>
+__device__ __forceinline__ Wave16qState wave16q_setup(const NetDev &nd, _Float16 *buf, const float4 *mlp, const uint16_t *tab, const half8 *w0, int lane)
+{
+    Wave16qState st;
+    st.lane = lane;
+    if constexpr (LEVEL >= 1) { wave16q_fill<1>(st, nd, mlp, tab, w0); wave16q_fill<6>(st, nd, mlp, tab, w0); }
+    if constexpr (LEVEL >= 2) wave16q_fill<2>(st, nd, mlp, tab, w0);
+    if constexpr (LEVEL >= 3) wave16q_fill<3>(st, nd, mlp, tab, w0);
+    if (lane < CS16) {
+#pragma unroll
+        for (int p = 0; p < 4; ++p) buf[p * PLANE16 + PIX * CS16 + lane] = (_Float16)0.0f;
+    }
+    return st;
+}
+template <int LEVEL, bool SANITISE = false, bool MLPEARLY = false>
+__device__ __forceinline__ void wave16q_pass(const Wave16qState &st0, const NetDev &nd, _Float16 *buf, const float4 *mlp, const float *bias_lds,
+                                             const uint16_t *tab, uint64_t b0, uint64_t b1, float *__restrict__ values,
+                                             float *__restrict__ priors, int out, const half8 *w0, unsigned long long *stamps = nullptr,
+                                             uint32_t *bad = nullptr)
+{
+    Wave16qState st = st0;
+    const int lane = st.lane;
     const int n = lane & 15, g = lane >> 4;
     auto stamp = [&](int i) { if (stamps && lane == 0) stamps[i] = __builtin_amdgcn_s_memtime(); };
     stamp(0);
     _Float16 *const p0h = buf, *const p0l = buf + PLANE16, *const p1h = buf + 2 * PLANE16, *const p1l = buf + 3 * PLANE16;
-    const __amdgpu_buffer_rsrc_t wr = wq_rsrc(nd);
-    const int voff = lane * 16;
+    if constexpr (LEVEL < 1) wave16q_fill<1>(st, nd, mlp, tab, w0);
+    const __amdgpu_buffer_rsrc_t wr = st.wr;
+    const int voff = st.voff;
     int soff = 2 * 4096;
     half8 wh[WTAPS][2], wl[WTAPS][2];
 #pragma unroll
@@ -768,13 +828,9 @@
     half8 swh[4], swl[4];
 #pragma unroll
     for (int i = 0; i < 4; ++i) { swh[i] = w0[(W0_STEM + i) * 64 + lane]; swl[i] = w0[(W0_STEM + 4 + i) * 64 + lane]; }
-    const float hb0 = nd.head_b[0], hb1 = nd.head_b[1], hb2 = nd.head_b[2];
-    uint32_t tb[TAB16 / 2];
-    {
-        const uint4 *t4 = reinterpret_cast<const uint4 *>(tab + lane * TAB16);
-#pragma unroll
-        for (int i = 0; i < TAB16 / 8; ++i) { const uint4 v = t4[i]; tb[4 * i] = v.x; tb[4 * i + 1] = v.y; tb[4 * i + 2] = v.z; tb[4 * i + 3] = v.w; }
-    }
+    const float hb0 = st.hb0, hb1 = st.hb1, hb2 = st.hb2;
+    if constexpr (LEVEL < 2) wave16q_fill<2>(st, nd, mlp, tab, w0);
+    const uint32_t (&tb)[TAB16 / 2] = st.tb;
     auto tof = [&](int idx) -> int { return (int)((tb[idx >> 1] >> (16 * (idx & 1))) & 0xffffu); };
     _Float16 *inp = p1h;
     if (lane <= PIX) {
@@ -788,17 +844,8 @@
         }
         *reinterpret_cast<half4 *>(inp + lane * 4) = v;
     }
-    if (lane < CS16) {
-        p0h[PIX * CS16 + lane] = (_Float16)0.0f; p0l[PIX * CS16 + lane] = (_Float16)0.0f;
-        p1h[PIX * CS16 + lane] = (_Float16)0.0f; p1l[PIX * CS16 + lane] = (_Float16)0.0f;
-    }
-    bool real[RT16];
-    int rbase[RT16];
-#pragma unroll
-    for (int rt = 0; rt < RT16; ++rt) {
-        real[rt] = 16 * rt + n < PIX;
-        rbase[rt] = (real[rt] ? 16 * rt + n : PIX) * CS16;
-    }
+    const bool (&real)[RT16] = st.real;
+    const int (&rbase)[RT16] = st.rbase;
     auto bias4 = [&](const float *b, int ct) -> floatx4 {
         const float4 v = *reinterpret_cast<const float4 *>(b + 16 * ct + 4 * g);
         return floatx4{v.x, v.y, v.z, v.w};
@@ -906,8 +953,11 @@
 #pragma unroll
                 for (int ct = 0; ct < 2; ++ct) {
                     half8 idf;
-#pragma unroll
-                    for (int j = 0; j < 8; ++j) idf[j] = (_Float16)((8 * g + j) == 16 * ct + n ? 1.0f : 0.0f);
+                    if constexpr (LEVEL >= 3) idf = st.idf[ct];
+                    else {
+#pragma unroll
+                        for (int j = 0; j < 8; ++j) idf[j] = (_Float16)((8 * g + j) == 16 * ct + n ? 1.0f : 0.0f);
+                    }
                     ah[rt][ct] = __builtin_amdgcn_mfma_f32_16x16x32_f16(idf, xh, ah[rt][ct], 0, 0, 0);
                     al[rt][ct] = __builtin_amdgcn_mfma_f32_16x16x32_f16(idf, xl, al[rt][ct], 0, 0, 0);
                 }
@@ -926,6 +976,14 @@
         layer(std::true_type{}, 2 * blk + 1);
     }
     stamp(8);
+    const float *pt = reinterpret_cast<const float *>(mlp + VT_F4);
+    float4 mwv[11];
+    float mpw[11];
+    if constexpr (MLPEARLY) {
+#pragma unroll
+        for (int q = 0; q < 11; ++q) { mwv[q] = mlp[q * 64 + lane]; mpw[q] = pt[q * 64 + lane]; }
+        if constexpr (LEVEL < 1) wave16q_fill<6>(st, nd, mlp, tab, w0);
+    }
     float *hs = reinterpret_cast<float *>(p1h);
     {
         const half8 hwh = w0[W0_HEAD * 64 + lane], hwl = w0[(W0_HEAD + 1) * 64 + lane];
@@ -951,6 +1009,235 @@
     }
     stamp(9);
     {
+        const float4 *hA4 = reinterpret_cast<const float4 *>(hs);
+        float v0 = 0.0f;
+#pragma unroll
+        for (int q = 0; q < 11; ++q) {
+            const float4 wv = MLPEARLY ? mwv[q] : mlp[q * 64 + lane];
+            const float4 xa = hA4[q];
+            v0 += wv.x * xa.x + wv.y * xa.y + wv.z * xa.z + wv.w * xa.w;
+        }
+        const int seg = lane >> 3;
+        const float *hpA = hs + PIX + seg * 11;
+        float l0 = 0.0f;
+#pragma unroll
+        for (int cc0 = 0; cc0 < 11; ++cc0) {
+            const float wv = MLPEARLY ? mpw[cc0] : pt[cc0 * 64 + lane];
+            const int cc = seg * 11 + cc0 < 2 * PIX ? cc0 : 2 * PIX - 1 - seg * 11;
+            l0 += wv * hpA[cc];
+        }
+        l0 += dppf<0x128>(l0);
+#pragma unroll
+        for (int m = 16; m <= 32; m <<= 1) l0 += __shfl_xor(l0, m, 64);
+        if constexpr (LEVEL < 1 && !MLPEARLY) wave16q_fill<6>(st, nd, mlp, tab, w0);
+        const float fb = st.fb, vw = st.vw, pb = st.pb;
+        const bool is_pol = lane < 7;
+        const float a = v0 + fb;
+        const float lg = l0 + pb;
+        const float rs = sum16(lane < PIX ? vw * lrelu(a) : 0.0f);
+        const float vsum = readlane_f(rs, 0) + readlane_f(rs, 16) + readlane_f(rs, 32);
+        const float value = (tanhf(vsum + nd.vout_b) + nd.w1) * nd.w2;
+        const float mx = max8(is_pol ? lg : -INFINITY);
+        const float e = is_pol ? expf(lg - mx) : 0.0f;
+        const float sum = sum8(e);
+        const float prior = e / sum;
+        if constexpr (SANITISE) {
+            const bool bad_v = !(value >= 0.0f && value <= 1.0f), bad_p = is_pol && !(prior >= 0.0f && prior <= 3.0e38f);
+            if (lane == 0) values[out] = bad_v ? 0.5f : value;
+            if (is_pol) priors[(size_t)out * 7 + lane] = bad_p ? 0.0f : prior;
+            if (__builtin_amdgcn_ballot_w64(bad_v || bad_p) != 0 && lane == 0) atomicAdd(bad, 1u);
+        } else {
+            if (lane == 0) values[out] = value;
+            if (is_pol) priors[(size_t)out * 7 + lane] = prior;
+        }
+    }
+    stamp(10);
+}
+
+__device__ __forceinline__ void net_forward_wave16q(const NetDev &nd, _Float16 *buf, const float4 *mlp, const float *bias_lds,
+                                                    const uint16_t *tab, uint64_t b0, uint64_t b1, float *__restrict__ values,
+                                                    float *__restrict__ priors, int out, const half8 *w0, unsigned long long *stamps = nullptr)
+{
+    int lane_ = threadIdx.x & 63;
+    asm volatile("" : "+v"(lane_));
+    const Wave16qState st = wave16q_setup<0>(nd, buf, mlp, tab, w0, lane_);
+    wave16q_pass<0>(st, nd, buf, mlp, bias_lds, tab, b0, b1, values, priors, out, w0, stamps);
+}
+
+constexpr int CS64 = 72;
+constexpr int PLANE64 = PROWS * CS64;
+constexpr int WUNITS = 3;
+
+__device__ __forceinline__ void net_forward_wave16w(const NetDev &nd, _Float16 *buf, const float4 *mlp, const float *bias_lds,
+                                                    const uint16_t *tab, uint64_t b0, uint64_t b1, float *__restrict__ values,
+                                                    float *__restrict__ priors, int out, unsigned long long *stamps = nullptr)
+{
+    constexpr int FW = 64, CT = 4, KS = 2;
+    int lane_ = threadIdx.x & 63;
+    asm volatile("" : "+v"(lane_));
+    const int lane = lane_;
+    const int n = lane & 15, g = lane >> 4;
+    auto stamp = [&](int i) { if (stamps && lane == 0) stamps[i] = __builtin_amdgcn_s_memtime(); };
+    stamp(0);
+    const int n_layers = 2 * nd.n_res;
+    _Float16 *const p0 = buf, *const p1 = buf + PLANE64;
+    half8 w[WUNITS][CT];
+    const half8 *wp = nd.conv_w16 + lane;
+    const int total_units = n_layers * 18;
+#pragma unroll
+    for (int u = 0; u < WUNITS; ++u) {
+        const int U = u < total_units ? u : 0;
+#pragma unroll
+        for (int ct = 0; ct < CT; ++ct) w[u][ct] = wp[(U * CT + ct) * 64];
+    }
+    half8 sw[2][CT];
+#pragma unroll
+    for (int s = 0; s < 2; ++s)
+#pragma unroll
+        for (int ct = 0; ct < CT; ++ct) sw[s][ct] = nd.stem_w16[(s * CT + ct) * 64 + lane];
+    const half8 hw0 = nd.head_w16[lane], hw1 = nd.head_w16[64 + lane];
+    const float hb0 = nd.head_b[0], hb1 = nd.head_b[1], hb2 = nd.head_b[2];
+    uint32_t tb[TAB16 / 2];
+    {
+        const uint4 *t4 = reinterpret_cast<const uint4 *>(tab + lane * TAB16);
+#pragma unroll
+        for (int i = 0; i < TAB16 / 8; ++i) { const uint4 v = t4[i]; tb[4 * i] = v.x; tb[4 * i + 1] = v.y; tb[4 * i + 2] = v.z; tb[4 * i + 3] = v.w; }
+    }
+    auto tof = [&](int idx) -> int { return (int)((tb[idx >> 1] >> (16 * (idx & 1))) & 0xffffu); };
+    _Float16 *inp = p1;
+    if (lane <= PIX) {
+        half4 v = {};
+        if (lane < PIX) {
+            const int y = lane / 7, x = lane - y * 7;
+            const int bit = x * 7 + (5 - y);
+            v[0] = (_Float16)((__popcll(b0 | b1) & 1) ? 0.0f : 1.0f);
+            v[1] = (_Float16)(float)((b0 >> bit) & 1);
+            v[2] = (_Float16)(float)((b1 >> bit) & 1);
+        }
+        *reinterpret_cast<half4 *>(inp + lane * 4) = v;
+    }
+    for (int i = lane; i < CS64; i += 64) { p0[PIX * CS64 + i] = (_Float16)0.0f; p1[PIX * CS64 + i] = (_Float16)0.0f; }
+    bool real[RT16];
+    int rbase[RT16];
+#pragma unroll
+    for (int rt = 0; rt < RT16; ++rt) {
+        real[rt] = 16 * rt + n < PIX;
+        rbase[rt] = (real[rt] ? 16 * rt + n : PIX) * CS64;
+    }
+    auto bias4 = [&](const float *b, int ct) -> floatx4 {
+        const float4 v = *reinterpret_cast<const float4 *>(b + 16 * ct + 4 * g);
+        return floatx4{v.x, v.y, v.z, v.w};
+    };
+    {
+        floatx4 acc[RT16][CT];
+#pragma unroll
+        for (int ct = 0; ct < CT; ++ct) {
+            const floatx4 bv = bias4(bias_lds, ct);
+#pragma unroll
+            for (int rt = 0; rt < RT16; ++rt) acc[rt][ct] = bv;
+        }
+#pragma unroll
+        for (int s = 0; s < 2; ++s)
+#pragma unroll
+            for (int rt = 0; rt < RT16; ++rt) {
+                const half4 va = *reinterpret_cast<const half4 *>(inp + tof(27 + rt * 4 + s * 2));
+                const half4 vb = *reinterpret_cast<const half4 *>(inp + tof(27 + rt * 4 + s * 2 + 1));
+                half8 bf;
+#pragma unroll
+                for (int j = 0; j < 4; ++j) { bf[j] = va[j]; bf[4 + j] = vb[j]; }
+#pragma unroll
+                for (int ct = 0; ct < CT; ++ct) acc[rt][ct] = __builtin_amdgcn_mfma_f32_16x16x32_f16(sw[s][ct], bf, acc[rt][ct], 0, 0, 0);
+            }
+#pragma unroll
+        for (int rt = 0; rt < RT16; ++rt)
+#pragma unroll
+            for (int ct = 0; ct < CT; ++ct) store16(acc[rt][ct], p0, rbase[rt] + 16 * ct + 4 * g, real[rt]);
+    }
+    stamp(1);
+    auto layer = [&](auto second_tag, const int L) {
+        constexpr bool second = decltype(second_tag)::value;
+        const _Float16 *src = second ? p1 : p0;
+        _Float16 *dst = second ? p0 : p1;
+        floatx4 acc[RT16][CT];
+#pragma unroll
+        for (int ct = 0; ct < CT; ++ct) {
+            const floatx4 bv = bias4(bias_lds + FW * (1 + L), ct);
+#pragma unroll
+            for (int rt = 0; rt < RT16; ++rt) acc[rt][ct] = bv;
+        }
+        half8 bc[RT16], bn[RT16];
+#pragma unroll
+        for (int rt = 0; rt < RT16; ++rt) bc[rt] = *reinterpret_cast<const half8 *>(src + tof(rt * 9));
+#pragma unroll
+        for (int u = 0; u < 18; ++u) {
+            if (u + 1 < 18) {
+#pragma unroll
+                for (int rt = 0; rt < RT16; ++rt) bn[rt] = *reinterpret_cast<const half8 *>(src + tof(rt * 9 + (u + 1) / 2) + 32 * ((u + 1) % 2));
+            }
+#pragma unroll
+            for (int ct = 0; ct < CT; ++ct) {
+                const half8 cw = w[u % WUNITS][ct];
+#pragma unroll
+                for (int rt = 0; rt < RT16; ++rt) acc[rt][ct] = __builtin_amdgcn_mfma_f32_16x16x32_f16(cw, bc[rt], acc[rt][ct], 0, 0, 0);
+            }
+            {
+                int U = L * 18 + u + WUNITS;
+                U = U < total_units ? U : 0;
+#pragma unroll
+                for (int ct = 0; ct < CT; ++ct) w[u % WUNITS][ct] = wp[(U * CT + ct) * 64];
+            }
+#pragma unroll
+            for (int rt = 0; rt < RT16; ++rt) bc[rt] = bn[rt];
+        }
+        if (second) {
+#pragma unroll
+            for (int rt = 0; rt < RT16; ++rt)
+#pragma unroll
+                for (int ks = 0; ks < KS; ++ks) {
+                    const half8 x = *reinterpret_cast<const half8 *>(dst + rbase[rt] + 32 * ks + 8 * g);
+#pragma unroll
+                    for (int c2 = 0; c2 < 2; ++c2) {
+                        half8 idf;
+#pragma unroll
+                        for (int j = 0; j < 8; ++j) idf[j] = (_Float16)((8 * g + j) == 16 * c2 + n ? 1.0f : 0.0f);
+                        acc[rt][2 * ks + c2] = __builtin_amdgcn_mfma_f32_16x16x32_f16(idf, x, acc[rt][2 * ks + c2], 0, 0, 0);
+                    }
+                }
+        }
+#pragma unroll
+        for (int rt = 0; rt < RT16; ++rt)
+#pragma unroll
+            for (int ct = 0; ct < CT; ++ct) store16(acc[rt][ct], dst, rbase[rt] + 16 * ct + 4 * g, real[rt]);
+        if (L < 6) stamp(2 + L);
+    };
+    for (int blk = 0; blk < nd.n_res; ++blk) {
+        layer(std::false_type{}, 2 * blk);
+        layer(std::true_type{}, 2 * blk + 1);
+    }
+    stamp(8);
+    float *hs = reinterpret_cast<float *>(p1);
+    {
+        floatx4 a[RT16];
+#pragma unroll
+        for (int rt = 0; rt < RT16; ++rt) {
+            const half8 x0 = *reinterpret_cast<const half8 *>(p0 + rbase[rt] + 8 * g);
+            const half8 x1 = *reinterpret_cast<const half8 *>(p0 + rbase[rt] + 32 + 8 * g);
+            a[rt] = __builtin_amdgcn_mfma_f32_16x16x32_f16(hw0, x0, floatx4{0.0f, 0.0f, 0.0f, 0.0f}, 0, 0, 0);
+            a[rt] = __builtin_amdgcn_mfma_f32_16x16x32_f16(hw1, x1, a[rt], 0, 0, 0);
+        }
+#pragma unroll
+        for (int rt = 0; rt < RT16; ++rt) {
+            const int r = 16 * rt + n;
+            if (g == 0 && r < PIX) {
+                hs[0 * PIX + r] = lrelu(a[rt][0] + hb0);
+                hs[1 * PIX + r] = lrelu(a[rt][1] + hb1);
+                hs[2 * PIX + r] = lrelu(a[rt][2] + hb2);
+            }
+        }
+        if (lane < 2) hs[HEADV + lane] = 0.0f;
+    }
+    stamp(9);
+    {
         const float *vt_b = reinterpret_cast<const float *>(mlp + VT_F4 + PT_F / 4);
         const float *pt = reinterpret_cast<const float *>(mlp + VT_F4);
         const float4 *hA4 = reinterpret_cast<const float4 *>(hs);
@@ -965,9 +1252,9 @@
         const float *hpA = hs + PIX + seg * 11;
         float l0 = 0.0f;
 #pragma unroll
-        for (int cc0 = 0; cc0 < 11; ++cc0) {
-            const float wv = pt[cc0 * 64 + lane];
-            const int cc = seg * 11 + cc0 < 2 * PIX ? cc0 : 2 * PIX - 1 - seg * 11;
+        for (int c = 0; c < 11; ++c) {
+            const float wv = pt[c * 64 + lane];
+            const int cc = seg * 11 + c < 2 * PIX ? c : 2 * PIX - 1 - seg * 11;
             l0 += wv * hpA[cc];
         }
         l0 += dppf<0x128>(l0);
@@ -989,38 +1276,31 @@
     stamp(10);
 }
 
-constexpr int CS64 = 72;
-constexpr int PLANE64 = PROWS * CS64;
-constexpr int WUNITS = 3;
-
-__device__ __forceinline__ void net_forward_wave16w(const NetDev &nd, _Float16 *buf, const float4 *mlp, const float *bias_lds,
+__device__ __forceinline__ void net_forward_wave16x(const NetDev &nd, _Float16 *buf, const float4 *mlp, const float *bias_lds,
                                                     const uint16_t *tab, uint64_t b0, uint64_t b1, float *__restrict__ values,
                                                     float *__restrict__ priors, int out, unsigned long long *stamps = nullptr)
 {
-    constexpr int FW = 64, CT = 4, KS = 2;
+    constexpr int FW = 64;
     int lane_ = threadIdx.x & 63;
     asm volatile("" : "+v"(lane_));
     const int lane = lane_;
     const int n = lane & 15, g = lane >> 4;
     auto stamp = [&](int i) { if (stamps && lane == 0) stamps[i] = __builtin_amdgcn_s_memtime(); };
     stamp(0);
-    const int n_layers = 2 * nd.n_res;
-    _Float16 *const p0 = buf, *const p1 = buf + PLANE64;
-    half8 w[WUNITS][CT];
-    const half8 *wp = nd.conv_w16 + lane;
-    const int total_units = n_layers * 18;
-#pragma unroll
-    for (int u = 0; u < WUNITS; ++u) {
-        const int U = u < total_units ? u : 0;
-#pragma unroll
-        for (int ct = 0; ct < CT; ++ct) w[u][ct] = wp[(U * CT + ct) * 64];
-    }
-    half8 sw[2][CT];
-#pragma unroll
-    for (int s = 0; s < 2; ++s)
-#pragma unroll
-        for (int ct = 0; ct < CT; ++ct) sw[s][ct] = nd.stem_w16[(s * CT + ct) * 64 + lane];
-    const half8 hw0 = nd.head_w16[lane], hw1 = nd.head_w16[64 + lane];
+    _Float16 *const p0h = buf, *const p0l = buf + PLANE64, *const p1h = buf + 2 * PLANE64, *const p1l = buf + 3 * PLANE64;
+    const __amdgpu_buffer_rsrc_t wr = wq_rsrc(nd);
+    const int voff = lane * 16;
+    half8 wh[WTAPS][2], wl[WTAPS][2];
+#pragma unroll
+    for (int t = 0; t < 2; ++t)
+#pragma unroll
+        for (int ct = 0; ct < 2; ++ct) {
+            wh[t][ct] = wq_load(wr, voff + (2 * ct) * 1024, t * 4096);
+            wl[t][ct] = wq_load(wr, voff + (2 * ct + 1) * 1024, t * 4096);
+        }
+#pragma unroll
+    for (int ct = 0; ct < 2; ++ct) { wh[2][ct] = wh[0][ct]; wl[2][ct] = wl[0][ct]; }
+    int soff = 2 * 4096;
     const float hb0 = nd.head_b[0], hb1 = nd.head_b[1], hb2 = nd.head_b[2];
     uint32_t tb[TAB16 / 2];
     {
@@ -1029,7 +1309,7 @@
         for (int i = 0; i < TAB16 / 8; ++i) { const uint4 v = t4[i]; tb[4 * i] = v.x; tb[4 * i + 1] = v.y; tb[4 * i + 2] = v.z; tb[4 * i + 3] = v.w; }
     }
     auto tof = [&](int idx) -> int { return (int)((tb[idx >> 1] >> (16 * (idx & 1))) & 0xffffu); };
-    _Float16 *inp = p1;
+    _Float16 *inp = p1h;
     if (lane <= PIX) {
         half4 v = {};
         if (lane < PIX) {
@@ -1041,7 +1321,10 @@
         }
         *reinterpret_cast<half4 *>(inp + lane * 4) = v;
     }
-    for (int i = lane; i < CS64; i += 64) { p0[PIX * CS64 + i] = (_Float16)0.0f; p1[PIX * CS64 + i] = (_Float16)0.0f; }
+    for (int i = lane; i < CS64; i += 64) {
+        p0h[PIX * CS64 + i] = (_Float16)0.0f; p0l[PIX * CS64 + i] = (_Float16)0.0f;
+        p1h[PIX * CS64 + i] = (_Float16)0.0f; p1l[PIX * CS64 + i] = (_Float16)0.0f;
+    }
     bool real[RT16];
     int rbase[RT16];
 #pragma unroll
@@ -1053,13 +1336,23 @@
         const float4 v = *reinterpret_cast<const float4 *>(b + 16 * ct + 4 * g);
         return floatx4{v.x, v.y, v.z, v.w};
     };
-    {
-        floatx4 acc[RT16][CT];
-#pragma unroll
-        for (int ct = 0; ct < CT; ++ct) {
-            const floatx4 bv = bias4(bias_lds, ct);
-#pragma unroll
-            for (int rt = 0; rt < RT16; ++rt) acc[rt][ct] = bv;
+    const floatx4 zero4 = {0.0f, 0.0f, 0.0f, 0.0f};
+#pragma unroll 1
+    for (int ch = 0; ch < 2; ++ch) {
+        half8 swh[2][2], swl[2][2];
+#pragma unroll
+        for (int s = 0; s < 2; ++s)
+#pragma unroll
+            for (int ct = 0; ct < 2; ++ct) {
+                swh[s][ct] = nd.stem_w16[(s * 4 + 2 * ch + ct) * 64 + lane];
+                swl[s][ct] = nd.stem_w16l[(s * 4 + 2 * ch + ct) * 64 + lane];
+            }
+        floatx4 ah[RT16][2], al[RT16][2];
+#pragma unroll
+        for (int ct = 0; ct < 2; ++ct) {
+            const floatx4 bv = bias4(bias_lds + 32 * ch, ct);
+#pragma unroll
+            for (int rt = 0; rt < RT16; ++rt) { ah[rt][ct] = bv; al[rt][ct] = zero4; }
         }
 #pragma unroll
         for (int s = 0; s < 2; ++s)
@@ -1071,68 +1364,103 @@
 #pragma unroll
                 for (int j = 0; j < 4; ++j) { bf[j] = va[j]; bf[4 + j] = vb[j]; }
 #pragma unroll
-                for (int ct = 0; ct < CT; ++ct) acc[rt][ct] = __builtin_amdgcn_mfma_f32_16x16x32_f16(sw[s][ct], bf, acc[rt][ct], 0, 0, 0);
+                for (int ct = 0; ct < 2; ++ct) {
+                    ah[rt][ct] = __builtin_amdgcn_mfma_f32_16x16x32_f16(swh[s][ct], bf, ah[rt][ct], 0, 0, 0);
+                    al[rt][ct] = __builtin_amdgcn_mfma_f32_16x16x32_f16(swl[s][ct], bf, al[rt][ct], 0, 0, 0);
+                }
             }
 #pragma unroll
         for (int rt = 0; rt < RT16; ++rt)
 #pragma unroll
-            for (int ct = 0; ct < CT; ++ct) store16(acc[rt][ct], p0, rbase[rt] + 16 * ct + 4 * g, real[rt]);
+            for (int ct = 0; ct < 2; ++ct) store16q(ah[rt][ct], al[rt][ct], p0h, p0l, rbase[rt] + 32 * ch + 16 * ct + 4 * g, real[rt]);
     }
     stamp(1);
     auto layer = [&](auto second_tag, const int L) {
         constexpr bool second = decltype(second_tag)::value;
-        const _Float16 *src = second ? p1 : p0;
-        _Float16 *dst = second ? p0 : p1;
-        floatx4 acc[RT16][CT];
-#pragma unroll
-        for (int ct = 0; ct < CT; ++ct) {
-            const floatx4 bv = bias4(bias_lds + FW * (1 + L), ct);
-#pragma unroll
-            for (int rt = 0; rt < RT16; ++rt) acc[rt][ct] = bv;
-        }
-        half8 bc[RT16], bn[RT16];
-#pragma unroll
-        for (int rt = 0; rt < RT16; ++rt) bc[rt] = *reinterpret_cast<const half8 *>(src + tof(rt * 9));
-#pragma unroll
-        for (int u = 0; u < 18; ++u) {
-            if (u + 1 < 18) {
-#pragma unroll
-                for (int rt = 0; rt < RT16; ++rt) bn[rt] = *reinterpret_cast<const half8 *>(src + tof(rt * 9 + (u + 1) / 2) + 32 * ((u + 1) % 2));
-            }
-#pragma unroll
-            for (int ct = 0; ct < CT; ++ct) {
-                const half8 cw = w[u % WUNITS][ct];
-#pragma unroll
-                for (int rt = 0; rt < RT16; ++rt) acc[rt][ct] = __builtin_amdgcn_mfma_f32_16x16x32_f16(cw, bc[rt], acc[rt][ct], 0, 0, 0);
-            }
-            {
-                int U = L * 18 + u + WUNITS;
-                U = U < total_units ? U : 0;
-#pragma unroll
-                for (int ct = 0; ct < CT; ++ct) w[u % WUNITS][ct] = wp[(U * CT + ct) * 64];
-            }
-#pragma unroll
-            for (int rt = 0; rt < RT16; ++rt) bc[rt] = bn[rt];
-        }
-        if (second) {
+        const _Float16 *sh = second ? p1h : p0h, *sl = second ? p1l : p0l;
+        _Float16 *dh = second ? p0h : p1h, *dl = second ? p0l : p1l;
+#pragma unroll 1
+        for (int ch = 0; ch < 2; ++ch) {
+            floatx4 ah[RT16][2], al[RT16][2];
+#pragma unroll
+            for (int ct = 0; ct < 2; ++ct) {
+                const floatx4 bv = bias4(bias_lds + FW * (1 + L) + 32 * ch, ct);
+#pragma unroll
+                for (int rt = 0; rt < RT16; ++rt) { ah[rt][ct] = bv; al[rt][ct] = zero4; }
+            }
+            half8 bh[RT16], bl[RT16], nh[RT16], nl[RT16];
+#pragma unroll
+            for (int rt = 0; rt < RT16; ++rt) {
+                bh[rt] = *reinterpret_cast<const half8 *>(sh + tof(rt * 9));
+                bl[rt] = *reinterpret_cast<const half8 *>(sl + tof(rt * 9));
+            }
+#if C4_F32X3_SGB
+            __builtin_amdgcn_sched_barrier(0);
+#endif
+#pragma unroll
+            for (int u = 0; u < 18; ++u) {
+                {
+#pragma unroll
+                    for (int ct = 0; ct < 2; ++ct) {
+                        wh[(u + 2) % WTAPS][ct] = wq_load(wr, voff + (2 * ct) * 1024, soff);
+                        wl[(u + 2) % WTAPS][ct] = wq_load(wr, voff + (2 * ct + 1) * 1024, soff);
+                    }
+                    soff += 4096;
+                }
+                if (u + 1 < 18) {
+#pragma unroll
+                    for (int rt = 0; rt < RT16; ++rt) {
+                        nh[rt] = *reinterpret_cast<const half8 *>(sh + tof(rt * 9 + (u + 1) / 2) + 32 * ((u + 1) % 2));
+                        nl[rt] = *reinterpret_cast<const half8 *>(sl + tof(rt * 9 + (u + 1) / 2) + 32 * ((u + 1) % 2));
+                    }
+                }
+#pragma unroll
+                for (int ct = 0; ct < 2; ++ct) {
+                    const half8 cwh = wh[u % WTAPS][ct], cwl = wl[u % WTAPS][ct];
+#pragma unroll
+                    for (int rt = 0; rt < RT16; ++rt) {
+                        ah[rt][ct] = __builtin_amdgcn_mfma_f32_16x16x32_f16(cwh, bh[rt], ah[rt][ct], 0, 0, 0);
+                        al[rt][ct] = __builtin_amdgcn_mfma_f32_16x16x32_f16(cwl, bh[rt], al[rt][ct], 0, 0, 0);
+                        al[rt][ct] = __builtin_amdgcn_mfma_f32_16x16x32_f16(cwh, bl[rt], al[rt][ct], 0, 0, 0);
+                    }
+                }
+#pragma unroll
+                for (int rt = 0; rt < RT16; ++rt) { bh[rt] = nh[rt]; bl[rt] = nl[rt]; }
+#if C4_F32X3_SGB
+#pragma unroll
+                for (int i = 0; i < 4; ++i) { __builtin_amdgcn_sched_group_barrier(0x008, 1, 0); __builtin_amdgcn_sched_group_barrier(0x020, 1, 0); }
+                if (u + 1 < 18) {
+#pragma unroll
+                    for (int i = 0; i < 6; ++i) { __builtin_amdgcn_sched_group_barrier(0x008, 2, 0); __builtin_amdgcn_sched_group_barrier(0x100, 1, 0); }
+                    __builtin_amdgcn_sched_group_barrier(0x008, 2, 0);
+                } else {
+                    __builtin_amdgcn_sched_group_barrier(0x008, 14, 0);
+                }
+#endif
+            }
+#if C4_F32X3_SGB
+            __builtin_amdgcn_sched_barrier(0);
+#endif
+            if (second) {
+#pragma unroll
+                for (int rt = 0; rt < RT16; ++rt) {
+                    const half8 xh = *reinterpret_cast<const half8 *>(dh + rbase[rt] + 32 * ch + 8 * g);
+                    const half8 xl = *reinterpret_cast<const half8 *>(dl + rbase[rt] + 32 * ch + 8 * g);
+#pragma unroll
+                    for (int ct = 0; ct < 2; ++ct) {
+                        half8 idf;
+#pragma unroll
+                        for (int j = 0; j < 8; ++j) idf[j] = (_Float16)((8 * g + j) == 16 * ct + n ? 1.0f : 0.0f);
+                        ah[rt][ct] = __builtin_amdgcn_mfma_f32_16x16x32_f16(idf, xh, ah[rt][ct], 0, 0, 0);
+                        al[rt][ct] = __builtin_amdgcn_mfma_f32_16x16x32_f16(idf, xl, al[rt][ct], 0, 0, 0);
+                    }
+                }
+            }
 #pragma unroll
             for (int rt = 0; rt < RT16; ++rt)
 #pragma unroll
-                for (int ks = 0; ks < KS; ++ks) {
-                    const half8 x = *reinterpret_cast<const half8 *>(dst + rbase[rt] + 32 * ks + 8 * g);
-#pragma unroll
-                    for (int c2 = 0; c2 < 2; ++c2) {
-                        half8 idf;
-#pragma unroll
-                        for (int j = 0; j < 8; ++j) idf[j] = (_Float16)((8 * g + j) == 16 * c2 + n ? 1.0f : 0.0f);
-                        acc[rt][2 * ks + c2] = __builtin_amdgcn_mfma_f32_16x16x32_f16(idf, x, acc[rt][2 * ks + c2], 0, 0, 0);
-                    }
-                }
-        }
-#pragma unroll
-        for (int rt = 0; rt < RT16; ++rt)
-#pragma unroll
-            for (int ct = 0; ct < CT; ++ct) store16(acc[rt][ct], dst, rbase[rt] + 16 * ct + 4 * g, real[rt]);
+                for (int ct = 0; ct < 2; ++ct) store16q(ah[rt][ct], al[rt][ct], dh, dl, rbase[rt] + 32 * ch + 16 * ct + 4 * g, real[rt]);
+        }
         if (L < 6) stamp(2 + L);
     };
     for (int blk = 0; blk < nd.n_res; ++blk) {
@@ -1140,23 +1468,31 @@
         layer(std::true_type{}, 2 * blk + 1);
     }
     stamp(8);
-    float *hs = reinterpret_cast<float *>(p1);
-    {
-        floatx4 a[RT16];
+    float *hs = reinterpret_cast<float *>(p1h);
+    {
+        const half8 hwh0 = nd.head_w16[lane], hwh1 = nd.head_w16[64 + lane];
+        const half8 hwl0 = nd.head_w16l[lane], hwl1 = nd.head_w16l[64 + lane];
+        floatx4 a[RT16], b[RT16];
 #pragma unroll
         for (int rt = 0; rt < RT16; ++rt) {
-            const half8 x0 = *reinterpret_cast<const half8 *>(p0 + rbase[rt] + 8 * g);
-            const half8 x1 = *reinterpret_cast<const half8 *>(p0 + rbase[rt] + 32 + 8 * g);
-            a[rt] = __builtin_amdgcn_mfma_f32_16x16x32_f16(hw0, x0, floatx4{0.0f, 0.0f, 0.0f, 0.0f}, 0, 0, 0);
-            a[rt] = __builtin_amdgcn_mfma_f32_16x16x32_f16(hw1, x1, a[rt], 0, 0, 0);
+            const half8 xh0 = *reinterpret_cast<const half8 *>(p0h + rbase[rt] + 8 * g);
+            const half8 xl0 = *reinterpret_cast<const half8 *>(p0l + rbase[rt] + 8 * g);
+            const half8 xh1 = *reinterpret_cast<const half8 *>(p0h + rbase[rt] + 32 + 8 * g);
+            const half8 xl1 = *reinterpret_cast<const half8 *>(p0l + rbase[rt] + 32 + 8 * g);
+            a[rt] = __builtin_amdgcn_mfma_f32_16x16x32_f16(hwh0, xh0, zero4, 0, 0, 0);
+            a[rt] = __builtin_amdgcn_mfma_f32_16x16x32_f16(hwh1, xh1, a[rt], 0, 0, 0);
+            b[rt] = __builtin_amdgcn_mfma_f32_16x16x32_f16(hwl0, xh0, zero4, 0, 0, 0);
+            b[rt] = __builtin_amdgcn_mfma_f32_16x16x32_f16(hwh0, xl0, b[rt], 0, 0, 0);
+            b[rt] = __builtin_amdgcn_mfma_f32_16x16x32_f16(hwl1, xh1, b[rt], 0, 0, 0);
+            b[rt] = __builtin_amdgcn_mfma_f32_16x16x32_f16(hwh1, xl1, b[rt], 0, 0, 0);
         }
 #pragma unroll
         for (int rt = 0; rt < RT16; ++rt) {
             const int r = 16 * rt + n;
             if (g == 0 && r < PIX) {
-                hs[0 * PIX + r] = lrelu(a[rt][0] + hb0);
-                hs[1 * PIX + r] = lrelu(a[rt][1] + hb1);
-                hs[2 * PIX + r] = lrelu(a[rt][2] + hb2);
+                hs[0 * PIX + r] = lrelu(a[rt][0] + b[rt][0] * LO_INV + hb0);
+                hs[1 * PIX + r] = lrelu(a[rt][1] + b[rt][1] * LO_INV + hb1);
+                hs[2 * PIX + r] = lrelu(a[rt][2] + b[rt][2] * LO_INV + hb2);
             }
         }
         if (lane < 2) hs[HEADV + lane] = 0.0f;
@@ -1201,267 +1537,6 @@
     stamp(10);
 }
 
-__device__ __forceinline__ void net_forward_wave16x(const NetDev &nd, _Float16 *buf, const float4 *mlp, const float *bias_lds,
-                                                    const uint16_t *tab, uint64_t b0, uint64_t b1, float *__restrict__ values,
-                                                    float *__restrict__ priors, int out, unsigned long long *stamps = nullptr)
-{
-    constexpr int FW = 64;
-    int lane_ = threadIdx.x & 63;
-    asm volatile("" : "+v"(lane_));
-    const int lane = lane_;
-    const int n = lane & 15, g = lane >> 4;
-    auto stamp = [&](int i) { if (stamps && lane == 0) stamps[i] = __builtin_amdgcn_s_memtime(); };
-    stamp(0);
-    _Float16 *const p0h = buf, *const p0l = buf + PLANE64, *const p1h = buf + 2 * PLANE64, *const p1l = buf + 3 * PLANE64;
-    const __amdgpu_buffer_rsrc_t wr = wq_rsrc(nd);
-    const int voff = lane * 16;
-    half8 wh[WTAPS][2], wl[WTAPS][2];
-#pragma unroll
-    for (int t = 0; t < 2; ++t)
-#pragma unroll
-        for (int ct = 0; ct < 2; ++ct) {
-            wh[t][ct] = wq_load(wr, voff + (2 * ct) * 1024, t * 4096);
-            wl[t][ct] = wq_load(wr, voff + (2 * ct + 1) * 1024, t * 4096);
-        }
-#pragma unroll
-    for (int ct = 0; ct < 2; ++ct) { wh[2][ct] = wh[0][ct]; wl[2][ct] = wl[0][ct]; }
-    int soff = 2 * 4096;
-    const float hb0 = nd.head_b[0], hb1 = nd.head_b[1], hb2 = nd.head_b[2];
-    uint32_t tb[TAB16 / 2];
-    {
-        const uint4 *t4 = reinterpret_cast<const uint4 *>(tab + lane * TAB16);
-#pragma unroll
-        for (int i = 0; i < TAB16 / 8; ++i) { const uint4 v = t4[i]; tb[4 * i] = v.x; tb[4 * i + 1] = v.y; tb[4 * i + 2] = v.z; tb[4 * i + 3] = v.w; }
-    }
-    auto tof = [&](int idx) -> int { return (int)((tb[idx >> 1] >> (16 * (idx & 1))) & 0xffffu); };
-    _Float16 *inp = p1h;
-    if (lane <= PIX) {
-        half4 v = {};
-        if (lane < PIX) {
-            const int y = lane / 7, x = lane - y * 7;
-            const int bit = x * 7 + (5 - y);
-            v[0] = (_Float16)((__popcll(b0 | b1) & 1) ? 0.0f : 1.0f);
-            v[1] = (_Float16)(float)((b0 >> bit) & 1);
-            v[2] = (_Float16)(float)((b1 >> bit) & 1);
-        }
-        *reinterpret_cast<half4 *>(inp + lane * 4) = v;
-    }
-    for (int i = lane; i < CS64; i += 64) {
-        p0h[PIX * CS64 + i] = (_Float16)0.0f; p0l[PIX * CS64 + i] = (_Float16)0.0f;
-        p1h[PIX * CS64 + i] = (_Float16)0.0f; p1l[PIX * CS64 + i] = (_Float16)0.0f;
-    }
-    bool real[RT16];
-    int rbase[RT16];
-#pragma unroll
-    for (int rt = 0; rt < RT16; ++rt) {
-        real[rt] = 16 * rt + n < PIX;
-        rbase[rt] = (real[rt] ? 16 * rt + n : PIX) * CS64;
-    }
-    auto bias4 = [&](const float *b, int ct) -> floatx4 {
-        const float4 v = *reinterpret_cast<const float4 *>(b + 16 * ct + 4 * g);
-        return floatx4{v.x, v.y, v.z, v.w};
-    };
-    const floatx4 zero4 = {0.0f, 0.0f, 0.0f, 0.0f};
-#pragma unroll 1
-    for (int ch = 0; ch < 2; ++ch) {
-        half8 swh[2][2], swl[2][2];
-#pragma unroll
-        for (int s = 0; s < 2; ++s)
-#pragma unroll
-            for (int ct = 0; ct < 2; ++ct) {
-                swh[s][ct] = nd.stem_w16[(s * 4 + 2 * ch + ct) * 64 + lane];
-                swl[s][ct] = nd.stem_w16l[(s * 4 + 2 * ch + ct) * 64 + lane];
-            }
-        floatx4 ah[RT16][2], al[RT16][2];
-#pragma unroll
-        for (int ct = 0; ct < 2; ++ct) {
-            const floatx4 bv = bias4(bias_lds + 32 * ch, ct);
-#pragma unroll
-            for (int rt = 0; rt < RT16; ++rt) { ah[rt][ct] = bv; al[rt][ct] = zero4; }
-        }
-#pragma unroll
-        for (int s = 0; s < 2; ++s)
-#pragma unroll
-            for (int rt = 0; rt < RT16; ++rt) {
-                const half4 va = *reinterpret_cast<const half4 *>(inp + tof(27 + rt * 4 + s * 2));
-                const half4 vb = *reinterpret_cast<const half4 *>(inp + tof(27 + rt * 4 + s * 2 + 1));
-                half8 bf;
-#pragma unroll
-                for (int j = 0; j < 4; ++j) { bf[j] = va[j]; bf[4 + j] = vb[j]; }
-#pragma unroll
-                for (int ct = 0; ct < 2; ++ct) {
-                    ah[rt][ct] = __builtin_amdgcn_mfma_f32_16x16x32_f16(swh[s][ct], bf, ah[rt][ct], 0, 0, 0);
-                    al[rt][ct] = __builtin_amdgcn_mfma_f32_16x16x32_f16(swl[s][ct], bf, al[rt][ct], 0, 0, 0);
-                }
-            }
-#pragma unroll
-        for (int rt = 0; rt < RT16; ++rt)
-#pragma unroll
-            for (int ct = 0; ct < 2; ++ct) store16q(ah[rt][ct], al[rt][ct], p0h, p0l, rbase[rt] + 32 * ch + 16 * ct + 4 * g, real[rt]);
-    }
-    stamp(1);
-    auto layer = [&](auto second_tag, const int L) {
-        constexpr bool second = decltype(second_tag)::value;
-        const _Float16 *sh = second ? p1h : p0h, *sl = second ? p1l : p0l;
-        _Float16 *dh = second ? p0h : p1h, *dl = second ? p0l : p1l;
-#pragma unroll 1
-        for (int ch = 0; ch < 2; ++ch) {
-            floatx4 ah[RT16][2], al[RT16][2];
-#pragma unroll
-            for (int ct = 0; ct < 2; ++ct) {
-                const floatx4 bv = bias4(bias_lds + FW * (1 + L) + 32 * ch, ct);
-#pragma unroll
-                for (int rt = 0; rt < RT16; ++rt) { ah[rt][ct] = bv; al[rt][ct] = zero4; }
-            }
-            half8 bh[RT16], bl[RT16], nh[RT16], nl[RT16];
-#pragma unroll
-            for (int rt = 0; rt < RT16; ++rt) {
-                bh[rt] = *reinterpret_cast<const half8 *>(sh + tof(rt * 9));
-                bl[rt] = *reinterpret_cast<const half8 *>(sl + tof(rt * 9));
-            }
-#if C4_F32X3_SGB
-            __builtin_amdgcn_sched_barrier(0);
-#endif
-#pragma unroll
-            for (int u = 0; u < 18; ++u) {
-                {
-#pragma unroll
-                    for (int ct = 0; ct < 2; ++ct) {
-                        wh[(u + 2) % WTAPS][ct] = wq_load(wr, voff + (2 * ct) * 1024, soff);
-                        wl[(u + 2) % WTAPS][ct] = wq_load(wr, voff + (2 * ct + 1) * 1024, soff);
-                    }
-                    soff += 4096;
-                }
-                if (u + 1 < 18) {
-#pragma unroll
-                    for (int rt = 0; rt < RT16; ++rt) {
-                        nh[rt] = *reinterpret_cast<const half8 *>(sh + tof(rt * 9 + (u + 1) / 2) + 32 * ((u + 1) % 2));
-                        nl[rt] = *reinterpret_cast<const half8 *>(sl + tof(rt * 9 + (u + 1) / 2) + 32 * ((u + 1) % 2));
-                    }
-                }
-#pragma unroll
-                for (int ct = 0; ct < 2; ++ct) {
-                    const half8 cwh = wh[u % WTAPS][ct], cwl = wl[u % WTAPS][ct];
-#pragma unroll
-                    for (int rt = 0; rt < RT16; ++rt) {
-                        ah[rt][ct] = __builtin_amdgcn_mfma_f32_16x16x32_f16(cwh, bh[rt], ah[rt][ct], 0, 0, 0);
-                        al[rt][ct] = __builtin_amdgcn_mfma_f32_16x16x32_f16(cwl, bh[rt], al[rt][ct], 0, 0, 0);
-                        al[rt][ct] = __builtin_amdgcn_mfma_f32_16x16x32_f16(cwh, bl[rt], al[rt][ct], 0, 0, 0);
-                    }
-                }
-#pragma unroll
-                for (int rt = 0; rt < RT16; ++rt) { bh[rt] = nh[rt]; bl[rt] = nl[rt]; }
-#if C4_F32X3_SGB
-#pragma unroll
-                for (int i = 0; i < 4; ++i) { __builtin_amdgcn_sched_group_barrier(0x008, 1, 0); __builtin_amdgcn_sched_group_barrier(0x020, 1, 0); }
-                if (u + 1 < 18) {
-#pragma unroll
-                    for (int i = 0; i < 6; ++i) { __builtin_amdgcn_sched_group_barrier(0x008, 2, 0); __builtin_amdgcn_sched_group_barrier(0x100, 1, 0); }
-                    __builtin_amdgcn_sched_group_barrier(0x008, 2, 0);
-                } else {
-                    __builtin_amdgcn_sched_group_barrier(0x008, 14, 0);
-                }
-#endif
-            }
-#if C4_F32X3_SGB
-            __builtin_amdgcn_sched_barrier(0);
-#endif
-            if (second) {
-#pragma unroll
-                for (int rt = 0; rt < RT16; ++rt) {
-                    const half8 xh = *reinterpret_cast<const half8 *>(dh + rbase[rt] + 32 * ch + 8 * g);
-                    const half8 xl = *reinterpret_cast<const half8 *>(dl + rbase[rt] + 32 * ch + 8 * g);
-#pragma unroll
-                    for (int ct = 0; ct < 2; ++ct) {
-                        half8 idf;
-#pragma unroll
-                        for (int j = 0; j < 8; ++j) idf[j] = (_Float16)((8 * g + j) == 16 * ct + n ? 1.0f : 0.0f);
-                        ah[rt][ct] = __builtin_amdgcn_mfma_f32_16x16x32_f16(idf, xh, ah[rt][ct], 0, 0, 0);
-                        al[rt][ct] = __builtin_amdgcn_mfma_f32_16x16x32_f16(idf, xl, al[rt][ct], 0, 0, 0);
-                    }
-                }
-            }
-#pragma unroll
-            for (int rt = 0; rt < RT16; ++rt)
-#pragma unroll
-                for (int ct = 0; ct < 2; ++ct) store16q(ah[rt][ct], al[rt][ct], dh, dl, rbase[rt] + 32 * ch + 16 * ct + 4 * g, real[rt]);
-        }
-        if (L < 6) stamp(2 + L);
-    };
-    for (int blk = 0; blk < nd.n_res; ++blk) {
-        layer(std::false_type{}, 2 * blk);
-        layer(std::true_type{}, 2 * blk + 1);
-    }
-    stamp(8);
-    float *hs = reinterpret_cast<float *>(p1h);
-    {
-        const half8 hwh0 = nd.head_w16[lane], hwh1 = nd.head_w16[64 + lane];
-        const half8 hwl0 = nd.head_w16l[lane], hwl1 = nd.head_w16l[64 + lane];
-        floatx4 a[RT16], b[RT16];
-#pragma unroll
-        for (int rt = 0; rt < RT16; ++rt) {
-            const half8 xh0 = *reinterpret_cast<const half8 *>(p0h + rbase[rt] + 8 * g);
-            const half8 xl0 = *reinterpret_cast<const half8 *>(p0l + rbase[rt] + 8 * g);
-            const half8 xh1 = *reinterpret_cast<const half8 *>(p0h + rbase[rt] + 32 + 8 * g);
-            const half8 xl1 = *reinterpret_cast<const half8 *>(p0l + rbase[rt] + 32 + 8 * g);
-            a[rt] = __builtin_amdgcn_mfma_f32_16x16x32_f16(hwh0, xh0, zero4, 0, 0, 0);
-            a[rt] = __builtin_amdgcn_mfma_f32_16x16x32_f16(hwh1, xh1, a[rt], 0, 0, 0);
-            b[rt] = __builtin_amdgcn_mfma_f32_16x16x32_f16(hwl0, xh0, zero4, 0, 0, 0);
-            b[rt] = __builtin_amdgcn_mfma_f32_16x16x32_f16(hwh0, xl0, b[rt], 0, 0, 0);
-            b[rt] = __builtin_amdgcn_mfma_f32_16x16x32_f16(hwl1, xh1, b[rt], 0, 0, 0);
-            b[rt] = __builtin_amdgcn_mfma_f32_16x16x32_f16(hwh1, xl1, b[rt], 0, 0, 0);
-        }
-#pragma unroll
-        for (int rt = 0; rt < RT16; ++rt) {
-            const int r = 16 * rt + n;
-            if (g == 0 && r < PIX) {
-                hs[0 * PIX + r] = lrelu(a[rt][0] + b[rt][0] * LO_INV + hb0);
-                hs[1 * PIX + r] = lrelu(a[rt][1] + b[rt][1] * LO_INV + hb1);
-                hs[2 * PIX + r] = lrelu(a[rt][2] + b[rt][2] * LO_INV + hb2);
-            }
-        }
-        if (lane < 2) hs[HEADV + lane] = 0.0f;
-    }
-    stamp(9);
-    {
-        const float *vt_b = reinterpret_cast<const float *>(mlp + VT_F4 + PT_F / 4);
-        const float *pt = reinterpret_cast<const float *>(mlp + VT_F4);
-        const float4 *hA4 = reinterpret_cast<const float4 *>(hs);
-        float v0 = 0.0f;
-#pragma unroll
-        for (int q = 0; q < 11; ++q) {
-            const float4 wv = mlp[q * 64 + lane];
-            const float4 xa = hA4[q];
-            v0 += wv.x * xa.x + wv.y * xa.y + wv.z * xa.z + wv.w * xa.w;
-        }
-        const int seg = lane >> 3;
-        const float *hpA = hs + PIX + seg * 11;
-        float l0 = 0.0f;
-#pragma unroll
-        for (int c = 0; c < 11; ++c) {
-            const float wv = pt[c * 64 + lane];
-            const int cc = seg * 11 + c < 2 * PIX ? c : 2 * PIX - 1 - seg * 11;
-            l0 += wv * hpA[cc];
-        }
-        l0 += dppf<0x128>(l0);
-#pragma unroll
-        for (int m = 16; m <= 32; m <<= 1) l0 += __shfl_xor(l0, m, 64);
-        const float fb = vt_b[lane], vw = vt_b[64 + lane], pb = vt_b[128 + lane];
-        const bool is_pol = lane < 7;
-        const float a = v0 + fb;
-        const float lg = l0 + pb;
-        const float rs = sum16(lane < PIX ? vw * lrelu(a) : 0.0f);
-        const float vsum = readlane_f(rs, 0) + readlane_f(rs, 16) + readlane_f(rs, 32);
-        const float value = (tanhf(vsum + nd.vout_b) + nd.w1) * nd.w2;
-        const float mx = max8(is_pol ? lg : -INFINITY);
-        const float e = is_pol ? expf(lg - mx) : 0.0f;
-        const float sum = sum8(e);
-        if (lane == 0) values[out] = value;
-        if (is_pol) priors[(size_t)out * 7 + lane] = e / sum;
-    }
-    stamp(10);
-}
-
 constexpr int NETMODE_F32_F16 = 0;
 constexpr int NETMODE_F32_PRECISE = 1;
 constexpr int NETMODE_F64 = 2;
```
